# Apokleos/kata-xpu-device-plugin

Measured on AMD Instinct MI355X. Metric: Allocate() p50 latency, lower is better.
Workload: dtype n/a; 1 GPU; model=kata-xpu-device-plugin-amd pod-churn, node=8x MI355X (mock sysfs, vfio-pci), gpus_per_pod=1, discovered_gpus=8, concurrent_clients=1, parallelism=1 churn client(s), one plugin daemon

## Files before the change

### kata_xpu_device_plugin_amd/config.py

```python
from __future__ import annotations

import argparse
import dataclasses
import os
from dataclasses import dataclass, field
from typing import Optional, Sequence

STRATEGY_CDI_CRI = "cdi-cri"
STRATEGY_CDI_ANNOTATIONS = "cdi-annotations"
STRATEGY_DEVICE_NODES = "device-nodes"
STRATEGIES = (STRATEGY_CDI_CRI, STRATEGY_CDI_ANNOTATIONS, STRATEGY_DEVICE_NODES)

DEFAULT_VENDOR_ALLOWLIST = (0x1002,)


def bundled_pci_ids_path() -> str:
    return os.path.join(os.path.dirname(os.path.abspath(__file__)),
                        "data", "pci.ids")


def _env(name: str, default: str) -> str:
    return os.environ.get(f"KXDP_{name}", default)


def _env_int(name: str, default: int) -> int:
    return int(os.environ.get(f"KXDP_{name}", default))


def _env_float(name: str, default: float) -> float:
    return float(os.environ.get(f"KXDP_{name}", default))


def _env_bool(name: str, default: bool) -> bool:
    raw = os.environ.get(f"KXDP_{name}")
    if raw is None:
        return default
    return raw.strip().lower() in ("1", "true", "yes", "on")


@dataclass
class Config:
    sysfs_root: str = field(default_factory=lambda: _env("SYSFS_ROOT", "/sys"))
    dev_root: str = field(default_factory=lambda: _env("DEV_ROOT", "/dev"))

    vendor_allowlist: Sequence[int] = field(
        default_factory=lambda: tuple(
            int(v, 16) for v in _env("VENDORS", "1002").split(",") if v
        )
    )
    device_allowlist: Sequence[int] = field(
        default_factory=lambda: tuple(
            int(v, 16) for v in _env("DEVICES", "").split(",") if v
        )
    )
    required_driver: str = field(default_factory=lambda: _env("DRIVER", "vfio-pci"))
    gpu_class_prefixes: Sequence[int] = (0x03, 0x12)

    resource_namespace: str = field(default_factory=lambda: _env("NAMESPACE", "amd.com"))
    pci_ids_paths: Sequence[str] = field(
        default_factory=lambda: tuple(
            p for p in _env(
                "PCI_IDS",
                bundled_pci_ids_path()
                + ":/usr/share/misc/pci.ids:/usr/share/hwdata/pci.ids:/usr/pci.ids",
            ).split(":")
            if p
        )
    )
    unified_resource_name: str = field(default_factory=lambda: _env("UNIFIED_RESOURCE", ""))

    cdi_dir: str = field(default_factory=lambda: _env("CDI_DIR", "/var/run/cdi"))
    cdi_kind: str = field(default_factory=lambda: _env("CDI_KIND", "amd.com/gpu"))
    cdi_spec_name: str = field(default_factory=lambda: _env("CDI_SPEC_NAME", "kxdp-vfio"))
    cdi_format: str = field(default_factory=lambda: _env("CDI_FORMAT", "yaml"))
    cdi_version: str = field(default_factory=lambda: _env("CDI_VERSION", "0.8.0"))
    device_list_strategy: str = field(default_factory=lambda: _env("STRATEGY", STRATEGY_CDI_CRI))

    kubelet_socket_dir: str = field(
        default_factory=lambda: _env("KUBELET_DIR", "/var/lib/kubelet/device-plugins")
    )
    kubelet_socket_name: str = "kubelet.sock"
    plugin_socket_prefix: str = field(default_factory=lambda: _env("SOCKET_PREFIX", "kata-xpu-amd"))
    registration_mode: str = field(default_factory=lambda: _env("REGISTRATION_MODE", "legacy"))
    plugins_registry_dir: str = field(
        default_factory=lambda: _env("PLUGINS_REGISTRY", "/var/lib/kubelet/plugins_registry")
    )
    grpc_timeout_s: float = field(default_factory=lambda: _env_float("GRPC_TIMEOUT_S", 5.0))

    topology_hint_path: str = field(
        default_factory=lambda: _env("TOPOLOGY_HINT", "/etc/kata-xpu-amd/topology.json")
    )

    health_poll_interval_s: float = field(default_factory=lambda: _env_float("HEALTH_POLL_S", 10.0))
    amdsmi_health: bool = field(default_factory=lambda: _env_bool("AMDSMI_HEALTH", True))
    reject_unhealthy: bool = field(default_factory=lambda: _env_bool("REJECT_UNHEALTHY", True))
    gpu_probe_interval_s: float = field(default_factory=lambda: _env_float("GPU_PROBE_S", 0.0))
    rescan_interval_s: float = field(default_factory=lambda: _env_float("RESCAN_S", 0.0))

    rpc_timing_path: str = field(default_factory=lambda: _env("RPC_TIMING", ""))

    gc_tuning: bool = field(default_factory=lambda: _env_bool("GC_TUNING", True))
    cpu_affinity: str = field(default_factory=lambda: _env("CPU_AFFINITY", ""))

    metrics_port: int = field(default_factory=lambda: _env_int("METRICS_PORT", 0))
    log_level: str = field(default_factory=lambda: _env("LOG_LEVEL", "INFO"))

    native: str = field(default_factory=lambda: _env("NATIVE", "auto"))
    grpc_server: str = field(default_factory=lambda: _env("GRPC_SERVER", "auto"))

    def validate(self) -> None:
        if self.device_list_strategy not in STRATEGIES:
            raise ValueError(
                f"device_list_strategy must be one of {STRATEGIES}, "
                f"got {self.device_list_strategy!r}"
            )
        if self.cdi_format not in ("yaml", "json"):
            raise ValueError(f"cdi_format must be yaml|json, got {self.cdi_format!r}")
        from .cdi.schema import KNOWN_CDI_VERSIONS
        if self.cdi_version not in KNOWN_CDI_VERSIONS:
            raise ValueError(
                f"cdi_version must be one of {KNOWN_CDI_VERSIONS}, "
                f"got {self.cdi_version!r}")
        if "/" not in self.cdi_kind:
            raise ValueError(f"cdi_kind must look like vendor/class, got {self.cdi_kind!r}")
        if self.native not in ("auto", "require", "off"):
            raise ValueError(f"native must be auto|require|off, got {self.native!r}")
        if self.grpc_server not in ("auto", "native", "aio"):
            raise ValueError(
                f"grpc_server must be auto|native|aio, got {self.grpc_server!r}")
        if self.registration_mode not in ("legacy", "watcher", "both"):
            raise ValueError(
                f"registration_mode must be legacy|watcher|both, "
                f"got {self.registration_mode!r}")

    @property
    def kubelet_socket(self) -> str:
        return os.path.join(self.kubelet_socket_dir, self.kubelet_socket_name)

    @classmethod
    def add_args(cls, parser: argparse.ArgumentParser) -> None:
        g = parser.add_argument_group("plugin config (env: KXDP_*)")
        g.add_argument("--sysfs-root", dest="sysfs_root")
        g.add_argument("--dev-root", dest="dev_root")
        g.add_argument("--cdi-dir", dest="cdi_dir")
        g.add_argument("--cdi-kind", dest="cdi_kind")
        g.add_argument("--strategy", dest="device_list_strategy", choices=STRATEGIES)
        g.add_argument("--kubelet-dir", dest="kubelet_socket_dir")
        g.add_argument("--namespace", dest="resource_namespace")
        g.add_argument("--driver", dest="required_driver")
        g.add_argument("--topology-hint", dest="topology_hint_path")
        g.add_argument("--metrics-port", dest="metrics_port", type=int)
        g.add_argument("--log-level", dest="log_level")
        g.add_argument("--native", dest="native", choices=("auto", "require", "off"))
        g.add_argument("--grpc-server", dest="grpc_server",
                       choices=("auto", "native", "aio"))
        g.add_argument("--registration-mode", dest="registration_mode",
                       choices=("legacy", "watcher", "both"))
        g.add_argument("--plugins-registry", dest="plugins_registry_dir")
        g.add_argument("--unified-resource", dest="unified_resource_name")
        g.add_argument("--cdi-format", dest="cdi_format", choices=("yaml", "json"))
        g.add_argument("--gpu-probe-interval", dest="gpu_probe_interval_s",
                       type=float)

    @classmethod
    def from_args(cls, args: Optional[argparse.Namespace] = None) -> "Config":
        cfg = cls()
        if args is not None:
            for f in dataclasses.fields(cls):
                v = getattr(args, f.name, None)
                if v is not None:
                    setattr(cfg, f.name, v)
        cfg.validate()
        return cfg
```

### kata_xpu_device_plugin_amd/plugin/server.py

```python
from __future__ import annotations

import asyncio
import atexit
import os
import threading
import time
import weakref
from typing import Dict, List, Optional

import grpc
import grpc.aio

from ..cdi.spec import ANNOTATION_PREFIX, qualified_name
from ..config import Config, STRATEGY_CDI_ANNOTATIONS, STRATEGY_CDI_CRI
from ..discovery.sysfs import read_hex, read_link_base
from ..topology.hive import GPUTopology, preferred_sets
from ..utils.log import get_logger
from . import api
from .state import DeviceState

log = get_logger(__name__)

try:
    from .. import _native as _NATIVE
except ImportError:
    _NATIVE = None

ENV_CDI_VENDOR_CLASS = "KUBERNETES_CDI_VENDOR_CLASS"
ENV_PCI_RESOURCE_PREFIX = "PCI_RESOURCE_"

_DEVICE_PLUGIN_PATH = "/v1beta1.DevicePlugin/"

_LIVE_NATIVE = weakref.WeakSet()


@atexit.register
def _stop_native_servers() -> None:
    for plugin in list(_LIVE_NATIVE):
        srv = plugin._native_server
        if srv is not None:
            try:
                srv.stop(0.0)
            except Exception:
                pass


def _stream_open() -> None:
    """DeviceState subscription of one open native ListAndWatch stream."""


def native_server_available() -> bool:
    return _NATIVE is not None and hasattr(_NATIVE, "GrpcServer")


class AllocationError(Exception):
    pass


class XPUDevicePlugin:

    def __init__(
        self,
        cfg: Config,
        resource_name: str,
        state: DeviceState,
        topo: GPUTopology,
        socket_name: Optional[str] = None,
    ):
        self.cfg = cfg
        self.resource_name = resource_name
        self.state = state
        self.topo = topo
        short = resource_name.split("/", 1)[1].lower()
        self.socket_name = socket_name or f"{cfg.plugin_socket_prefix}-{short}.sock"
        self.socket_path = os.path.join(cfg.kubelet_socket_dir, self.socket_name)
        self._aio_server: Optional[grpc.aio.Server] = None
        self._loop: Optional[asyncio.AbstractEventLoop] = None
        self._thread: Optional[threading.Thread] = None
        self._stop = threading.Event()
        self._serving = threading.Event()
        self._lifecycle = threading.Lock()
        self._removal_lock = threading.Lock()
        self._expected_removals = 0
        self.watcher_servicer = None
        self.watcher_socket_path: Optional[str] = None
        self._allocations = 0
        self._allocate_failures = 0
        self._last_allocate_s = 0.0
        self._allocate_seconds_total = 0.0
        self._native_server = None
        self._native_unsubscribe = None
        self._stream_subscriptions: List = []
        self._devices_dir = os.path.join(cfg.sysfs_root, "bus", "pci", "devices")
        self._vendor_list = list(cfg.vendor_allowlist)
        self._qn_cache: Dict[str, str] = {}
        self._bdf_cache = None
        self._timing = {"allocate_us": [], "preferred_us": [],
                        "loop_lag_us": []} if cfg.rpc_timing_path else None
        self._env_res_name = ENV_PCI_RESOURCE_PREFIX + resource_name.upper(
        ).replace("/", "_").replace(".", "_").replace("-", "_")

    def _native_stats(self):
        srv = self._native_server
        return srv.stats() if srv is not None else (0, 0, None, 0.0)

    @property
    def allocations(self) -> int:
        return self._allocations + self._native_stats()[0]

    @allocations.setter
    def allocations(self, v: int) -> None:
        self._allocations = v

    @property
    def allocate_failures(self) -> int:
        return self._allocate_failures + self._native_stats()[1]

    @allocate_failures.setter
    def allocate_failures(self, v: int) -> None:
        self._allocate_failures = v

    @property
    def last_allocate_s(self) -> float:
        last = self._native_stats()[2]
        return self._last_allocate_s if not last else last

    @last_allocate_s.setter
    def last_allocate_s(self, v: float) -> None:
        self._last_allocate_s = v

    @property
    def allocate_seconds_total(self) -> float:
        return self._allocate_seconds_total + self._native_stats()[3]

    @allocate_seconds_total.setter
    def allocate_seconds_total(self, v: float) -> None:
        self._allocate_seconds_total = v

    def _qn(self, gid: str) -> str:
        qn = self._qn_cache.get(gid)
        if qn is None:
            qn = self._qn_cache[gid] = qualified_name(self.cfg.cdi_kind, gid)
        return qn

    async def GetDevicePluginOptions(self, request, context):
        return api.DevicePluginOptions(
            pre_start_required=False,
            get_preferred_allocation_available=True,
        )

    def _device_list(self, snapshot=None) -> List[object]:
        devs = []
        if snapshot is None:
            snapshot = self.state.snapshot()
        for dev, healthy in snapshot:
            d = api.Device(
                id=dev.id,
                health=api.HEALTHY if healthy else api.UNHEALTHY,
            )
            if dev.numa_node >= 0:
                d.topology.nodes.add(id=dev.numa_node)
            devs.append(d)
        return devs

    async def ListAndWatch(self, request, context):
        loop = asyncio.get_running_loop()
        event = asyncio.Event()

        def _notify() -> None:
            try:
                loop.call_soon_threadsafe(event.set)
            except RuntimeError:
                pass

        unsubscribe = self.state.subscribe(_notify)
        try:
            yield api.ListAndWatchResponse(devices=self._device_list())
            while not self._stop.is_set():
                await event.wait()
                event.clear()
                if self._stop.is_set():
                    break
                yield api.ListAndWatchResponse(devices=self._device_list())
        finally:
            unsubscribe()

    def _revalidate_many(self, ids: List[str]) -> None:
        groups = []
        for gid in ids:
            dev = self.state.device(gid)
            if dev is None:
                raise AllocationError(f"unknown device id {gid}")
            if self.cfg.reject_unhealthy and not self.state.is_healthy(gid):
                raise AllocationError(f"device {gid} is Unhealthy")
            groups.append((gid, [fn.bdf for fn in dev.functions]))
        if self.cfg.native != "off":
            if _NATIVE is None and self.cfg.native == "require":
                raise RuntimeError("_native extension required but missing")
            if _NATIVE is not None:
                err = _NATIVE.revalidate_groups(
                    self._devices_dir, groups,
                    self._vendor_list, self.cfg.required_driver,
                )
                if err:
                    raise AllocationError(err)
                return
        for gid, _bdfs in groups:
            self._revalidate_py(gid)

    def _revalidate_py(self, gid: str) -> None:
        dev = self.state.device(gid)
        assert dev is not None
        devices_dir = self._devices_dir
        for fn in dev.functions:
            p = os.path.join(devices_dir, fn.bdf)
            if read_link_base(os.path.join(p, "iommu_group")) != gid:
                raise AllocationError(f"device {fn.bdf} no longer in IOMMU group {gid}")
            vendor = read_hex(os.path.join(p, "vendor"))
            if vendor not in set(self.cfg.vendor_allowlist):
                raise AllocationError(f"device {fn.bdf} vendor {vendor:#x} not allowed")
            if read_link_base(os.path.join(p, "driver")) != self.cfg.required_driver:
                raise AllocationError(
                    f"device {fn.bdf} not bound to {self.cfg.required_driver}"
                )

    def _container_response(self, ids: List[str]):
        resp = api.ContainerAllocateResponse()
        strategy = self.cfg.device_list_strategy
        bdfs: List[str] = []
        if ids and strategy not in (STRATEGY_CDI_CRI, STRATEGY_CDI_ANNOTATIONS):
            vfio_ctl = os.path.join(self.cfg.dev_root, "vfio", "vfio")
            resp.devices.add(
                container_path=vfio_ctl, host_path=vfio_ctl, permissions="rw"
            )
        for gid in ids:
            dev = self.state.device(gid)
            assert dev is not None
            bdfs.extend(dev.bdfs)
            if strategy == STRATEGY_CDI_CRI:
                resp.cdi_devices.add(name=self._qn(gid))
            elif strategy == STRATEGY_CDI_ANNOTATIONS:
                key = f"{ANNOTATION_PREFIX}vfio{gid}"
                resp.annotations[key] = self._qn(gid)
            else:
                path = os.path.join(self.cfg.dev_root, dev.vfio_node)
                resp.devices.add(
                    container_path=path, host_path=path, permissions="rw"
                )
        if strategy in (STRATEGY_CDI_CRI, STRATEGY_CDI_ANNOTATIONS):
            resp.envs[ENV_CDI_VENDOR_CLASS] = self.cfg.cdi_kind
        resp.envs[self._env_res_name] = ",".join(bdfs)
        return resp

    async def Allocate(self, request, context):
        t0 = time.perf_counter()
        response = api.AllocateResponse()
        try:
            for creq in request.container_requests:
                ids = list(creq.devices_ids)
                self._revalidate_many(ids)
                response.container_responses.append(self._container_response(ids))
        except AllocationError as e:
            self.allocate_failures += 1
            log.warning("Allocate(%s) rejected: %s", self.resource_name, e)
            await context.abort(grpc.StatusCode.INVALID_ARGUMENT, str(e))
        self.allocations += 1
        self.last_allocate_s = time.perf_counter() - t0
        self.allocate_seconds_total += self.last_allocate_s
        if self._timing is not None:
            self._timing["allocate_us"].append(self.last_allocate_s * 1e6)
        return response

    async def GetPreferredAllocation(self, request, context):
        return self._preferred_allocation(request)

    def _preferred_allocation(self, request):
        t0 = time.perf_counter() if self._timing is not None else 0.0
        resp = api.PreferredAllocationResponse()
        gen = self.state.generation
        cached = self._bdf_cache
        if cached is not None and cached[0] == gen:
            bdf_of = cached[1]
        else:
            bdf_of = self.state.bdf_map()
            self._bdf_cache = (gen, bdf_of)
        for creq in request.container_requests:
            available = [d for d in creq.available_device_ids if d in bdf_of]
            must = list(creq.must_include_device_ids)
            pick = preferred_sets(
                self.topo, bdf_of, available, must, creq.allocation_size
            )
            resp.container_responses.add(device_ids=pick)
        if self._timing is not None:
            self._timing["preferred_us"].append(
                (time.perf_counter() - t0) * 1e6)
        return resp

    async def PreStartContainer(self, request, context):
        return api.PreStartContainerResponse()

    def start(self, register: bool = True) -> None:
        with self._lifecycle:
            self._start_locked(register)

    def _use_native_server(self) -> bool:
        want = self.cfg.grpc_server
        if want == "aio":
            return False
        if native_server_available() and self.cfg.native != "off":
            return True
        if want == "native":
            raise RuntimeError(
                "grpc_server=native needs the _native extension "
                "(and native != off)")
        if self.cfg.native == "require":
            raise RuntimeError("_native extension required but missing")
        return False

    def _start_locked(self, register: bool) -> None:
        self._stop.clear()
        if self._use_native_server():
            self._start_native()
        else:
            self._start_aio()
        ch = grpc.insecure_channel(f"unix://{self.socket_path}")
        try:
            grpc.channel_ready_future(ch).result(timeout=self.cfg.grpc_timeout_s)
        finally:
            ch.close()
        self._serving.set()
        if register and self.cfg.registration_mode in ("legacy", "both"):
            try:
                self.register_with_kubelet()
            except Exception as e:
                log.warning("kubelet registration failed (%s); serving "
                            "anyway and retrying in background", e)
                self._spawn_registration_retry()
        log.info("plugin %s serving on %s (%s registration)",
                 self.resource_name, self.socket_path,
                 self.cfg.registration_mode)

    def _start_aio(self) -> None:
        self._loop_ready = threading.Event()
        self._start_error: Optional[BaseException] = None
        self._thread = threading.Thread(
            target=self._serve_thread,
            name=f"kxdp-grpc-{self.resource_name.split('/')[-1]}",
            daemon=True,
        )
        self._thread.start()
        if not self._loop_ready.wait(self.cfg.grpc_timeout_s):
            raise RuntimeError(f"gRPC server for {self.resource_name} "
                               "did not start in time")
        if self._start_error is not None:
            self._thread.join(timeout=2.0)
            raise self._start_error

    def _start_native(self) -> None:
        os.makedirs(self.cfg.kubelet_socket_dir, exist_ok=True)
        if os.path.exists(self.socket_path):
            self._note_expected_removal()
            os.unlink(self.socket_path)
        paths = [self.socket_path]
        if self.cfg.registration_mode in ("watcher", "both"):
            from .watcher_registration import (
                SERVICE_PATH_PREFIX,
                WatcherRegistrationServicer,
            )
            os.makedirs(self.cfg.plugins_registry_dir, exist_ok=True)
            self.watcher_servicer = WatcherRegistrationServicer(
                self.resource_name, self.socket_path)
            self.watcher_socket_path = os.path.join(
                self.cfg.plugins_registry_dir, self.socket_name)
            if os.path.exists(self.watcher_socket_path):
                os.unlink(self.watcher_socket_path)
            paths.append(self.watcher_socket_path)
        srv = _NATIVE.GrpcServer(paths)
        p = _DEVICE_PLUGIN_PATH
        srv.register_constant(
            p + "GetDevicePluginOptions",
            api.DevicePluginOptions(
                pre_start_required=False,
                get_preferred_allocation_available=True,
            ).SerializeToString())
        srv.register_constant(
            p + "PreStartContainer",
            api.PreStartContainerResponse().SerializeToString())
        srv.register_watch(p + "ListAndWatch", self._on_watch_streams)
        srv.register_unary(p + "GetPreferredAllocation",
                           self._preferred_allocation_bytes)
        srv.configure_allocate(
            p + "Allocate",
            strategy=self.cfg.device_list_strategy,
            reject_unhealthy=bool(self.cfg.reject_unhealthy),
            cdi_kind=self.cfg.cdi_kind,
            env_name=self._env_res_name,
            dev_root=self.cfg.dev_root,
            devices_dir=self._devices_dir,
            vendors=self._vendor_list,
            required_driver=self.cfg.required_driver,
            on_reject=self._log_rejection,
            timing=self._timing is not None,
        )
        if self.watcher_servicer is not None and len(paths) > 1:
            srv.register_unary(SERVICE_PATH_PREFIX + "GetInfo",
                               self.watcher_servicer.get_info_bytes)
            srv.register_unary(
                SERVICE_PATH_PREFIX + "NotifyRegistrationStatus",
                self.watcher_servicer.notify_registration_status_bytes)
        self._native_server = srv
        self._native_unsubscribe = self.state.subscribe_snapshot(
            self._push_native_state)
        try:
            srv.start()
        except BaseException:
            self._native_unsubscribe()
            self._native_unsubscribe = None
            self._native_server = None
            raise
        _LIVE_NATIVE.add(self)

    def _push_native_state(self, snapshot, generation) -> None:
        srv = self._native_server
        if srv is None:
            return
        dev_root = self.cfg.dev_root
        rows = []
        for dev, healthy in snapshot:
            qn = self._qn(dev.id)
            rows.append((
                dev.id,
                [fn.bdf for fn in dev.functions],
                bool(healthy),
                api.CDIDevice(name=qn).SerializeToString(),
                f"{ANNOTATION_PREFIX}vfio{dev.id}",
                qn,
                os.path.join(dev_root, dev.vfio_node),
            ))
        srv.update_table(rows)
        srv.publish(api.ListAndWatchResponse(
            devices=self._device_list(snapshot)).SerializeToString())

    def _on_watch_streams(self, delta: int) -> None:
        subs = self._stream_subscriptions
        for _ in range(delta):
            subs.append(self.state.subscribe(_stream_open))
        for _ in range(-delta):
            if subs:
                subs.pop()()

    def _preferred_allocation_bytes(self, request: bytes) -> bytes:
        return self._preferred_allocation(
            api.PreferredAllocationRequest.FromString(request)
        ).SerializeToString()

    def _log_rejection(self, err: str) -> None:
        log.warning("Allocate(%s) rejected: %s", self.resource_name, err)

    def _stop_native(self) -> None:
        srv = self._native_server
        if srv is None:
            return
        if self._native_unsubscribe is not None:
            self._native_unsubscribe()
            self._native_unsubscribe = None
        srv.stop(1.0)
        n, fails, last, total = srv.stats()
        if self._timing is not None:
            self._timing["allocate_us"] = list(srv.allocate_timing_us())
            self._timing["loop_lag_us"] = []
            self._dump_timing()
        self._native_server = None
        _LIVE_NATIVE.discard(self)
        while self._stream_subscriptions:
            self._stream_subscriptions.pop()()
        self._allocations += n
        self._allocate_failures += fails
        self._allocate_seconds_total += total
        if last:
            self._last_allocate_s = last

    def _spawn_registration_retry(self) -> None:
        def retry():
            delay = 1.0
            while self._serving.is_set() and not self._stop.is_set():
                if self._stop.wait(delay):
                    return
                if not self._serving.is_set():
                    return
                try:
                    self.register_with_kubelet()
                    log.info("kubelet registration succeeded after retry")
                    return
                except Exception:
                    delay = min(delay * 2, 30.0)

        threading.Thread(target=retry, daemon=True,
                         name=f"kxdp-register-retry-{self.socket_name}").start()

    def _serve_thread(self) -> None:
        loop = asyncio.new_event_loop()
        self._loop = loop
        asyncio.set_event_loop(loop)

        async def _main():
            server = grpc.aio.server(
                options=[("grpc.max_concurrent_streams", 64),
                         ("grpc.optimization_target", "latency")])
            api.add_device_plugin_servicer(server, self)
            os.makedirs(self.cfg.kubelet_socket_dir, exist_ok=True)
            if os.path.exists(self.socket_path):
                self._note_expected_removal()
                os.unlink(self.socket_path)
            server.add_insecure_port(f"unix://{self.socket_path}")
            if self.cfg.registration_mode in ("watcher", "both"):
                from .watcher_registration import (
                    WatcherRegistrationServicer,
                    add_watcher_registration_servicer,
                )
                os.makedirs(self.cfg.plugins_registry_dir, exist_ok=True)
                self.watcher_servicer = WatcherRegistrationServicer(
                    self.resource_name, self.socket_path)
                self.watcher_socket_path = os.path.join(
                    self.cfg.plugins_registry_dir, self.socket_name)
                add_watcher_registration_servicer(server, self.watcher_servicer)
                if os.path.exists(self.watcher_socket_path):
                    os.unlink(self.watcher_socket_path)
                server.add_insecure_port(f"unix://{self.watcher_socket_path}")
            await server.start()
            self._aio_server = server
            self._stop_async = asyncio.Event()
            lag_task = None
            if self._timing is not None:
                async def _lag_monitor():
                    while not self._stop_async.is_set():
                        t0 = time.perf_counter()
                        await asyncio.sleep(0.001)
                        lag = (time.perf_counter() - t0 - 0.001) * 1e6
                        self._timing["loop_lag_us"].append(max(0.0, lag))
                        if len(self._timing["loop_lag_us"]) > 200_000:
                            del self._timing["loop_lag_us"][:100_000]
                lag_task = asyncio.ensure_future(_lag_monitor())
            self._loop_ready.set()
            await self._stop_async.wait()
            if lag_task is not None:
                lag_task.cancel()
            await server.stop(grace=1.0)
            if self._timing is not None:
                self._dump_timing()

        try:
            loop.run_until_complete(_main())
        except BaseException as e:
            self._start_error = e
            self._loop_ready.set()
        finally:
            try:
                loop.close()
            except Exception:
                pass

    def _dump_timing(self) -> None:
        import json
        import statistics as stats

        def dist(xs):
            if not xs:
                return None
            xs = sorted(xs)
            n = len(xs)
            return {"n": n,
                    "p50": round(xs[n // 2], 1),
                    "p90": round(xs[min(n - 1, int(n * 0.9))], 1),
                    "p99": round(xs[min(n - 1, int(n * 0.99))], 1),
                    "max": round(xs[-1], 1),
                    "mean": round(stats.fmean(xs), 1)}

        out = {k: dist(v) for k, v in self._timing.items()}
        path = f"{self.cfg.rpc_timing_path}.{self.socket_name}.json"
        try:
            with open(path, "w") as f:
                json.dump(out, f, indent=1)
            log.info("rpc timing breakdown → %s", path)
        except OSError as e:
            log.warning("could not write rpc timing: %s", e)

    def register_with_kubelet(self) -> None:
        ch = grpc.insecure_channel(f"unix://{self.cfg.kubelet_socket}")
        try:
            grpc.channel_ready_future(ch).result(timeout=self.cfg.grpc_timeout_s)
            stub = api.RegistrationStub(ch)
            stub.Register(
                api.RegisterRequest(
                    version=api.VERSION,
                    endpoint=self.socket_name,
                    resource_name=self.resource_name,
                    options=api.DevicePluginOptions(
                        pre_start_required=False,
                        get_preferred_allocation_available=True,
                    ),
                ),
                timeout=self.cfg.grpc_timeout_s,
            )
        finally:
            ch.close()

    def stop(self) -> None:
        with self._lifecycle:
            self._stop_locked()

    def _stop_locked(self) -> None:
        self._stop.set()
        self._serving.clear()
        self.state.poke()
        if os.path.exists(self.socket_path):
            self._note_expected_removal()
        self._stop_native()
        if self._loop is not None and getattr(self, "_stop_async", None) is not None:
            try:
                self._loop.call_soon_threadsafe(self._stop_async.set)
            except RuntimeError:
                pass
        if self._thread is not None:
            self._thread.join(timeout=5.0)
            self._thread = None
        self._aio_server = None
        self._loop = None
        for path in (self.socket_path,
                     getattr(self, "watcher_socket_path", None)):
            if path and os.path.exists(path):
                try:
                    os.unlink(path)
                except OSError:
                    pass

    def restart(self, register: bool = True) -> None:
        self.stop()
        self.start(register=register)

    def _note_expected_removal(self) -> None:
        with self._removal_lock:
            self._expected_removals += 1

    def consume_expected_removal(self) -> bool:
        with self._removal_lock:
            if self._expected_removals > 0:
                self._expected_removals -= 1
                return True
            return False

    @property
    def serving(self) -> bool:
        return self._serving.is_set()
```

### native/xpu_grpc_server.cpp

```cpp
#include <pybind11/pybind11.h>
#include <pybind11/stl.h>

#include <atomic>
#include <cerrno>
#include <chrono>
#include <cstring>
#include <fcntl.h>
#include <memory>
#include <mutex>
#include <poll.h>
#include <stdexcept>
#include <sys/epoll.h>
#include <sys/eventfd.h>
#include <sys/socket.h>
#include <sys/uio.h>
#include <sys/un.h>
#include <thread>
#include <unistd.h>
#include <unordered_map>

#include "h2.h"
#include "pbwire.h"

namespace py = pybind11;
using namespace kxdp;

namespace {

constexpr int STRATEGY_CDI_CRI = 0;
constexpr int STRATEGY_CDI_ANNOTATIONS = 1;
constexpr int STRATEGY_DEVICE_NODES = 2;
constexpr size_t kMaxTimingSamples = 1u << 20;

struct DeviceEntry {
    std::vector<std::string> bdfs;
    bool healthy = true;
    std::string cdi_device;
    std::string ann_key, ann_value;
    std::string dev_path;
};

using Table = std::unordered_map<std::string, DeviceEntry>;

struct AllocateConfig {
    bool enabled = false;
    std::string path;
    int strategy = STRATEGY_CDI_CRI;
    bool reject_unhealthy = true;
    std::string cdi_kind, env_name, dev_root, devices_dir, required_driver;
    std::vector<long> vendors;
    bool timing = false;
};

enum class Kind { CONSTANT, WATCH, PYTHON, ALLOCATE };

struct Method {
    Kind kind;
    std::string bytes;
    py::object fn;
};

std::string link_base(int dirfd, const char* name) {
    char buf[512];
    ssize_t n = ::readlinkat(dirfd, name, buf, sizeof(buf) - 1);
    if (n <= 0) return {};
    buf[n] = 0;
    const char* slash = std::strrchr(buf, '/');
    return std::string(slash ? slash + 1 : buf);
}

long read_vendor(int dirfd) {
    int fd = ::openat(dirfd, "vendor", O_RDONLY | O_CLOEXEC);
    if (fd < 0) return -1;
    char buf[64];
    ssize_t n = ::read(fd, buf, sizeof(buf) - 1);
    ::close(fd);
    if (n <= 0) return -1;
    buf[n] = 0;
    errno = 0;
    char* end = nullptr;
    long v = std::strtol(buf, &end, 16);
    if (errno || end == buf) return -1;
    return v;
}

struct IoConn {
    int fd;
    h2::Conn h2;
    size_t woff = 0;
    size_t watching = 0;
    bool want_write = false;
    IoConn(int f, h2::App* app) : fd(f), h2(app) {}
};

class GrpcServer : public h2::App {
public:
    explicit GrpcServer(std::vector<std::string> paths)
        : paths_(std::move(paths)) {}

    ~GrpcServer() override {
        if (thread_.joinable()) {
            py::gil_scoped_release rel;
            request_stop(0.0);
            thread_.join();
        }
        methods_.clear();
        on_reject_ = py::object();
        on_watch_change_ = py::object();
    }

    void register_constant(const std::string& path, const std::string& bytes) {
        check_not_running();
        methods_[path] = Method{Kind::CONSTANT, bytes, py::object()};
    }
    void register_watch(const std::string& path, py::object on_change) {
        check_not_running();
        methods_[path] = Method{Kind::WATCH, {}, py::object()};
        on_watch_change_ = std::move(on_change);
    }
    void register_unary(const std::string& path, py::object fn) {
        check_not_running();
        methods_[path] = Method{Kind::PYTHON, {}, std::move(fn)};
    }
    void configure_allocate(const std::string& path, const std::string& strategy,
                            bool reject_unhealthy, const std::string& cdi_kind,
                            const std::string& env_name,
                            const std::string& dev_root,
                            const std::string& devices_dir,
                            const std::vector<long>& vendors,
                            const std::string& required_driver,
                            py::object on_reject, bool timing) {
        check_not_running();
        alloc_.enabled = true;
        alloc_.path = path;
        alloc_.strategy = strategy == "cdi-cri" ? STRATEGY_CDI_CRI
                          : strategy == "cdi-annotations" ? STRATEGY_CDI_ANNOTATIONS
                          : STRATEGY_DEVICE_NODES;
        alloc_.reject_unhealthy = reject_unhealthy;
        alloc_.cdi_kind = cdi_kind;
        alloc_.env_name = env_name;
        alloc_.dev_root = dev_root;
        alloc_.devices_dir = devices_dir;
        alloc_.vendors = vendors;
        alloc_.required_driver = required_driver;
        alloc_.timing = timing;
        on_reject_ = std::move(on_reject);
        methods_[path] = Method{Kind::ALLOCATE, {}, py::object()};
    }

    void update_table(const std::vector<std::tuple<
            std::string, std::vector<std::string>, bool, py::bytes,
            std::string, std::string, std::string>>& devices) {
        auto t = std::make_shared<Table>();
        for (auto& d : devices) {
            DeviceEntry e;
            e.bdfs = std::get<1>(d);
            e.healthy = std::get<2>(d);
            e.cdi_device = std::string(std::get<3>(d));
            e.ann_key = std::get<4>(d);
            e.ann_value = std::get<5>(d);
            e.dev_path = std::get<6>(d);
            (*t)[std::get<0>(d)] = std::move(e);
        }
        std::lock_guard<std::mutex> g(table_mu_);
        table_ = std::move(t);
    }

    void publish(const std::string& message) {
        auto m = std::make_shared<const std::string>(message);
        {
            std::lock_guard<std::mutex> g(pub_mu_);
            latest_ = std::move(m);
            pub_gen_++;
        }
        wake();
    }

    void start() {
        if (thread_.joinable()) throw std::runtime_error("server already started");
        stop_.store(false);
        ep_ = ::epoll_create1(EPOLL_CLOEXEC);
        wake_fd_ = ::eventfd(0, EFD_NONBLOCK | EFD_CLOEXEC);
        if (ep_ < 0 || wake_fd_ < 0) {
            close_fds();
            throw std::runtime_error("epoll/eventfd setup failed");
        }
        add_epoll(wake_fd_, EPOLLIN);
        for (auto& path : paths_) {
            sockaddr_un addr{};
            addr.sun_family = AF_UNIX;
            if (path.size() >= sizeof(addr.sun_path)) {
                close_fds();
                throw std::runtime_error("socket path too long: " + path);
            }
            std::memcpy(addr.sun_path, path.c_str(), path.size() + 1);
            int fd = ::socket(AF_UNIX, SOCK_STREAM | SOCK_NONBLOCK | SOCK_CLOEXEC, 0);
            if (fd < 0 || ::bind(fd, (sockaddr*)&addr, sizeof(addr)) < 0 ||
                ::listen(fd, 128) < 0) {
                std::string why = std::strerror(errno);
                if (fd >= 0) ::close(fd);
                close_fds();
                throw std::runtime_error("cannot listen on " + path + ": " + why);
            }
            listeners_.push_back(fd);
            bound_.push_back(path);
            add_epoll(fd, EPOLLIN);
        }
        thread_ = std::thread([this] { run(); });
    }

    void stop(double grace) {
        if (!thread_.joinable()) return;
        py::gil_scoped_release rel;
        request_stop(grace);
        thread_.join();
    }

    bool running() const { return thread_.joinable(); }

    py::tuple stats() {
        std::lock_guard<std::mutex> g(stat_mu_);
        return py::make_tuple(allocations_, failures_, last_s_, total_s_);
    }

    std::vector<double> allocate_timing_us() {
        std::lock_guard<std::mutex> g(stat_mu_);
        return alloc_us_;
    }

    void on_rpc(h2::Conn& c, uint32_t sid, const std::string& path,
                std::string& msg) override {
        auto it = methods_.find(path);
        if (it == methods_.end())
            return c.reply_error(sid, h2::GRPC_UNIMPLEMENTED, "Method not found!");
        Method& m = it->second;
        switch (m.kind) {
        case Kind::CONSTANT:
            return c.reply_unary(sid, m.bytes);
        case Kind::ALLOCATE:
            return handle_allocate(c, sid, msg);
        case Kind::WATCH: {
            std::shared_ptr<const std::string> latest;
            {
                std::lock_guard<std::mutex> g(pub_mu_);
                latest = latest_;
            }
            c.start_stream(sid);
            if (latest) c.push_message(sid, *latest);
            return;
        }
        case Kind::PYTHON:
            return handle_python(c, sid, m, msg);
        }
    }

private:
    void check_not_running() {
        if (thread_.joinable())
            throw std::runtime_error("register methods before start()");
    }

    void wake() {
        if (wake_fd_ >= 0) {
            uint64_t one = 1;
            ssize_t r = ::write(wake_fd_, &one, sizeof(one));
            (void)r;
        }
    }

    void request_stop(double grace) {
        grace_s_ = grace;
        stop_.store(true);
        wake();
    }

    void add_epoll(int fd, uint32_t events) {
        epoll_event ev{};
        ev.events = events;
        ev.data.fd = fd;
        ::epoll_ctl(ep_, EPOLL_CTL_ADD, fd, &ev);
    }

    void close_fds() {
        for (int fd : listeners_) ::close(fd);
        listeners_.clear();
        for (auto& p : bound_) ::unlink(p.c_str());
        bound_.clear();
        if (wake_fd_ >= 0) ::close(wake_fd_);
        if (ep_ >= 0) ::close(ep_);
        wake_fd_ = ep_ = -1;
        if (dirfd_ >= 0) ::close(dirfd_);
        dirfd_ = -1;
        dirfd_table_ = nullptr;
    }

    struct GilHold {
        PyThreadState*& ts;
        bool held = false;
        explicit GilHold(PyThreadState*& t) : ts(t) {
            if (ts && !_Py_IsFinalizing()) {
                PyEval_RestoreThread(ts);
                held = true;
            }
        }
        ~GilHold() {
            if (held) ts = PyEval_SaveThread();
        }
    };

    void handle_python(h2::Conn& c, uint32_t sid, Method& m, std::string& msg) {
        bool ok = false;
        int status = h2::GRPC_UNKNOWN;
        std::string payload;
        {
            GilHold gil(ts_);
            if (!gil.held) {
                status = h2::GRPC_UNAVAILABLE;
                payload = "server shutting down";
            } else {
                try {
                    py::object r = m.fn(py::bytes(msg));
                    if (py::isinstance<py::bytes>(r)) {
                        payload = r.cast<std::string>();
                        ok = true;
                    } else {
                        auto t = r.cast<std::pair<int, std::string>>();
                        status = t.first;
                        payload = t.second;
                    }
                } catch (py::error_already_set& e) {
                    try {
                        payload = "Unexpected " +
                                  py::str(e.type()).cast<std::string>() + ": " +
                                  py::str(e.value()).cast<std::string>();
                    } catch (...) {
                        payload = "handler raised";
                    }
                    e.restore();
                    PyErr_Clear();
                } catch (std::exception& e) {
                    payload = e.what();
                }
            }
        }
        if (ok) c.reply_unary(sid, payload);
        else c.reply_error(sid, status, payload);
    }

    void report_watchers(IoConn& io, size_t now) {
        if (now == io.watching) return;
        long delta = (long)now - (long)io.watching;
        io.watching = now;
        GilHold gil(ts_);
        if (!gil.held || !on_watch_change_ || on_watch_change_.is_none()) return;
        try {
            on_watch_change_(delta);
        } catch (py::error_already_set& e) {
            e.restore();
            PyErr_Clear();
        }
    }

    void log_rejection(const std::string& err) {
        GilHold gil(ts_);
        if (!gil.held || !on_reject_ || on_reject_.is_none()) return;
        try {
            on_reject_(err);
        } catch (py::error_already_set& e) {
            e.restore();
            PyErr_Clear();
        }
    }

    bool open_devices_dir() {
        if (dirfd_ >= 0) ::close(dirfd_);
        dirfd_ = ::open(alloc_.devices_dir.c_str(),
                        O_RDONLY | O_DIRECTORY | O_CLOEXEC);
        return dirfd_ >= 0;
    }

    std::string revalidate(const std::string& gid, const DeviceEntry& dev) {
        for (const auto& bdf : dev.bdfs) {
            const int flags = O_RDONLY | O_DIRECTORY | O_CLOEXEC;
            int dfd = ::openat(dirfd_, bdf.c_str(), flags);
            if (dfd < 0) {
                if (!open_devices_dir())
                    return "cannot open " + alloc_.devices_dir;
                dfd = ::openat(dirfd_, bdf.c_str(), flags);
            }
            if (dfd < 0) return "device " + bdf + " vanished";
            std::string err;
            if (link_base(dfd, "iommu_group") != gid) {
                err = "device " + bdf + " no longer in IOMMU group " + gid;
            } else {
                long vendor = read_vendor(dfd);
                if (vendor < 0 ||
                    std::find(alloc_.vendors.begin(), alloc_.vendors.end(),
                              vendor) == alloc_.vendors.end())
                    err = "device " + bdf + " vendor not allowed";
                else if (link_base(dfd, "driver") != alloc_.required_driver)
                    err = "device " + bdf + " not bound to " +
                          alloc_.required_driver;
            }
            ::close(dfd);
            if (!err.empty()) return err;
        }
        return {};
    }

    std::string allocate_container(const Table& table,
                                   const std::vector<std::string>& ids,
                                   std::string& out) {
        std::vector<const DeviceEntry*> devs;
        devs.reserve(ids.size());
        for (const auto& gid : ids) {
            auto it = table.find(gid);
            if (it == table.end()) return "unknown device id " + gid;
            if (alloc_.reject_unhealthy && !it->second.healthy)
                return "device " + gid + " is Unhealthy";
            devs.push_back(&it->second);
        }
        if (dirfd_ < 0 || dirfd_table_ != &table) {
            if (!open_devices_dir()) return "cannot open " + alloc_.devices_dir;
            dirfd_table_ = &table;
        }
        for (size_t i = 0; i < ids.size(); i++) {
            std::string err = revalidate(ids[i], *devs[i]);
            if (!err.empty()) return err;
        }
        const bool cdi = alloc_.strategy != STRATEGY_DEVICE_NODES;
        std::string bdfs;
        for (auto* d : devs)
            for (const auto& b : d->bdfs) {
                if (!bdfs.empty()) bdfs.push_back(',');
                bdfs += b;
            }
        static const std::string kVendorClass = "KUBERNETES_CDI_VENDOR_CLASS";
        if (cdi && alloc_.env_name == kVendorClass) {
            pb::put_map_entry(out, 1, alloc_.env_name, bdfs);
        } else if (cdi && kVendorClass < alloc_.env_name) {
            pb::put_map_entry(out, 1, kVendorClass, alloc_.cdi_kind);
            pb::put_map_entry(out, 1, alloc_.env_name, bdfs);
        } else {
            pb::put_map_entry(out, 1, alloc_.env_name, bdfs);
            if (cdi) pb::put_map_entry(out, 1, kVendorClass, alloc_.cdi_kind);
        }
        if (!cdi) {
            auto spec = [&](const std::string& path) {
                std::string s;
                pb::put_bytes(s, 1, path);
                pb::put_bytes(s, 2, path);
                pb::put_bytes(s, 3, "rw", 2);
                pb::put_bytes(out, 3, s);
            };
            if (!ids.empty()) spec(alloc_.dev_root + "/vfio/vfio");
            for (auto* d : devs) spec(d->dev_path);
        }
        if (alloc_.strategy == STRATEGY_CDI_ANNOTATIONS)
            for (auto* d : devs)
                pb::put_map_entry(out, 4, d->ann_key, d->ann_value);
        if (alloc_.strategy == STRATEGY_CDI_CRI)
            for (auto* d : devs) pb::put_bytes(out, 5, d->cdi_device);
        return {};
    }

    void handle_allocate(h2::Conn& c, uint32_t sid, const std::string& msg) {
        auto t0 = std::chrono::steady_clock::now();
        std::shared_ptr<const Table> table;
        {
            std::lock_guard<std::mutex> g(table_mu_);
            table = table_;
        }
        std::vector<std::vector<std::string>> reqs;
        if (!pb::parse_allocate_request(msg, reqs))
            return c.reply_error(sid, h2::GRPC_INTERNAL,
                                 "Exception deserializing request!");
        static const Table kEmpty;
        const Table& tbl = table ? *table : kEmpty;
        std::string resp, err;
        for (const auto& ids : reqs) {
            std::string cresp;
            err = allocate_container(tbl, ids, cresp);
            if (!err.empty()) break;
            pb::put_bytes(resp, 1, cresp);
        }
        if (!err.empty()) {
            {
                std::lock_guard<std::mutex> g(stat_mu_);
                failures_++;
            }
            c.reply_error(sid, h2::GRPC_INVALID_ARGUMENT, err);
            log_rejection(err);
            return;
        }
        double dt = std::chrono::duration<double>(
                        std::chrono::steady_clock::now() - t0).count();
        {
            std::lock_guard<std::mutex> g(stat_mu_);
            allocations_++;
            last_s_ = dt;
            total_s_ += dt;
            if (alloc_.timing && alloc_us_.size() < kMaxTimingSamples)
                alloc_us_.push_back(dt * 1e6);
        }
        c.reply_unary(sid, resp);
    }

    void set_want_write(IoConn& io, bool on) {
        if (io.want_write == on) return;
        io.want_write = on;
        epoll_event ev{};
        ev.events = EPOLLIN | (on ? EPOLLOUT : 0);
        ev.data.fd = io.fd;
        ::epoll_ctl(ep_, EPOLL_CTL_MOD, io.fd, &ev);
    }

    bool flush(IoConn& io) {
        std::string& out = io.h2.out();
        while (io.woff < out.size()) {
            iovec iov{(void*)(out.data() + io.woff), out.size() - io.woff};
            msghdr mh{};
            mh.msg_iov = &iov;
            mh.msg_iovlen = 1;
            ssize_t n = ::sendmsg(io.fd, &mh, MSG_NOSIGNAL);
            if (n < 0) {
                if (errno == EINTR) continue;
                if (errno == EAGAIN || errno == EWOULDBLOCK) {
                    set_want_write(io, true);
                    return true;
                }
                return false;
            }
            io.woff += (size_t)n;
        }
        out.clear();
        io.woff = 0;
        set_want_write(io, false);
        return !io.h2.want_close();
    }

    void close_conn(int fd) {
        auto it = conns_.find(fd);
        if (it == conns_.end()) return;
        report_watchers(*it->second, 0);
        ::epoll_ctl(ep_, EPOLL_CTL_DEL, fd, nullptr);
        ::close(fd);
        conns_.erase(it);
    }

    void on_readable(IoConn& io) {
        ssize_t n = ::read(io.fd, rbuf_, sizeof(rbuf_));
        if (n == 0) return close_conn(io.fd);
        if (n < 0) {
            if (errno == EAGAIN || errno == EINTR) return;
            return close_conn(io.fd);
        }
        io.h2.feed((const uint8_t*)rbuf_, (size_t)n);
        report_watchers(io, io.h2.watch_streams());
        if (!flush(io)) close_conn(io.fd);
    }

    void deliver_publications() {
        std::shared_ptr<const std::string> latest;
        uint64_t gen;
        {
            std::lock_guard<std::mutex> g(pub_mu_);
            latest = latest_;
            gen = pub_gen_;
        }
        if (gen == pub_seen_ || !latest) return;
        pub_seen_ = gen;
        std::vector<int> done;
        for (auto& kv : conns_) {
            kv.second->h2.broadcast(*latest);
            if (!flush(*kv.second)) done.push_back(kv.first);
        }
        for (int fd : done) close_conn(fd);
    }

    void shutdown_connections() {
        for (int fd : listeners_) ::close(fd);
        listeners_.clear();
        for (auto& p : bound_) ::unlink(p.c_str());
        bound_.clear();
        for (auto& kv : conns_) kv.second->h2.begin_shutdown();
        auto deadline = std::chrono::steady_clock::now() +
                        std::chrono::duration<double>(grace_s_);
        for (auto& kv : conns_) {
            IoConn& io = *kv.second;
            while (flush(io) && io.woff < io.h2.out().size()) {
                auto left = std::chrono::duration_cast<std::chrono::milliseconds>(
                    deadline - std::chrono::steady_clock::now()).count();
                if (left <= 0) break;
                pollfd p{io.fd, POLLOUT, 0};
                if (::poll(&p, 1, (int)left) <= 0) break;
            }
            ::shutdown(io.fd, SHUT_WR);
            while (::read(io.fd, rbuf_, sizeof(rbuf_)) > 0) {}
            report_watchers(io, 0);
            ::close(io.fd);
        }
        conns_.clear();
    }

    void run() {
        PyGILState_STATE gstate = PyGILState_Ensure();
        ts_ = PyEval_SaveThread();
        epoll_event evs[64];
        while (!stop_.load()) {
            int n = ::epoll_wait(ep_, evs, 64, -1);
            if (n < 0) {
                if (errno == EINTR) continue;
                break;
            }
            for (int i = 0; i < n && !stop_.load(); i++) {
                int fd = evs[i].data.fd;
                if (fd == wake_fd_) {
                    uint64_t v;
                    while (::read(wake_fd_, &v, sizeof(v)) > 0) {}
                    deliver_publications();
                    continue;
                }
                if (std::find(listeners_.begin(), listeners_.end(), fd) !=
                    listeners_.end()) {
                    for (;;) {
                        int cfd = ::accept4(fd, nullptr, nullptr,
                                            SOCK_NONBLOCK | SOCK_CLOEXEC);
                        if (cfd < 0) break;
                        auto io = std::make_unique<IoConn>(cfd, this);
                        IoConn& ref = *io;
                        conns_[cfd] = std::move(io);
                        add_epoll(cfd, EPOLLIN);
                        if (!flush(ref)) close_conn(cfd);
                    }
                    continue;
                }
                auto it = conns_.find(fd);
                if (it == conns_.end()) continue;
                IoConn& io = *it->second;
                if (evs[i].events & EPOLLOUT) {
                    if (!flush(io)) {
                        close_conn(fd);
                        continue;
                    }
                }
                if (evs[i].events & (EPOLLIN | EPOLLHUP | EPOLLERR))
                    on_readable(io);
            }
        }
        shutdown_connections();
        if (!_Py_IsFinalizing()) {
            PyEval_RestoreThread(ts_);
            PyGILState_Release(gstate);
        }
        ts_ = nullptr;
        int ep = ep_, wfd = wake_fd_;
        ep_ = wake_fd_ = -1;
        ::close(ep);
        ::close(wfd);
        if (dirfd_ >= 0) ::close(dirfd_);
        dirfd_ = -1;
        dirfd_table_ = nullptr;
    }

    std::vector<std::string> paths_, bound_;
    std::unordered_map<std::string, Method> methods_;
    AllocateConfig alloc_;
    py::object on_reject_, on_watch_change_;

    std::mutex table_mu_;
    std::shared_ptr<const Table> table_;
    std::mutex pub_mu_;
    std::shared_ptr<const std::string> latest_;
    uint64_t pub_gen_ = 0;
    uint64_t pub_seen_ = 0;

    std::mutex stat_mu_;
    uint64_t allocations_ = 0, failures_ = 0;
    double last_s_ = 0.0, total_s_ = 0.0;
    std::vector<double> alloc_us_;

    std::thread thread_;
    std::atomic<bool> stop_{false};
    double grace_s_ = 1.0;
    int ep_ = -1, wake_fd_ = -1;
    std::vector<int> listeners_;
    std::unordered_map<int, std::unique_ptr<IoConn>> conns_;
    PyThreadState* ts_ = nullptr;
    int dirfd_ = -1;
    const Table* dirfd_table_ = nullptr;
    char rbuf_[65536];
};

}

void kxdp_init_grpc_server(py::module_& m) {
    py::class_<GrpcServer>(m, "GrpcServer")
        .def(py::init<std::vector<std::string>>(), py::arg("socket_paths"))
        .def("register_constant", &GrpcServer::register_constant,
             py::arg("path"), py::arg("response"))
        .def("register_watch", &GrpcServer::register_watch, py::arg("path"),
             py::arg("on_change") = py::none())
        .def("register_unary", &GrpcServer::register_unary, py::arg("path"),
             py::arg("fn"),
             "fn(request bytes) -> response bytes | (status code, message)")
        .def("configure_allocate", &GrpcServer::configure_allocate,
             py::arg("path"), py::arg("strategy"), py::arg("reject_unhealthy"),
             py::arg("cdi_kind"), py::arg("env_name"), py::arg("dev_root"),
             py::arg("devices_dir"), py::arg("vendors"),
             py::arg("required_driver"), py::arg("on_reject"),
             py::arg("timing") = false)
        .def("update_table", &GrpcServer::update_table, py::arg("devices"))
        .def("publish", &GrpcServer::publish, py::arg("message"))
        .def("start", &GrpcServer::start)
        .def("stop", &GrpcServer::stop, py::arg("grace") = 1.0)
        .def("stats", &GrpcServer::stats)
        .def("allocate_timing_us", &GrpcServer::allocate_timing_us)
        .def_property_readonly("running", &GrpcServer::running);
}
```

### setup.py

```python
import os
import subprocess
import sys

import pybind11

ROOT = os.path.dirname(os.path.abspath(__file__))
PKG = "kata_xpu_device_plugin_amd"


def build_hip(arch: str = "gfx950", verbose: bool = True) -> str:
    import sysconfig

    hipcc = os.environ.get("HIPCC", "/opt/rocm/bin/hipcc")
    src = os.path.join(ROOT, "probes", "xpu_probe.hip")
    ext = sysconfig.get_config_var("EXT_SUFFIX") or ".so"
    out = os.path.join(ROOT, PKG, f"_gpuprobe{ext}")
    if os.path.exists(out) and os.path.getmtime(out) > os.path.getmtime(src):
        return out
    cmd = [
        hipcc, f"--offload-arch={arch}", "-O3", "-std=c++17",
        "-fPIC", "-shared",
        "-x", "hip", src,
        f"-I{pybind11.get_include()}",
        f"-I{sysconfig.get_paths()['include']}",
        "-o", out,
    ]
    if verbose:
        print("+", " ".join(cmd), file=sys.stderr)
    subprocess.run(cmd, check=True)
    return out


if __name__ == "__main__" or "setuptools" in sys.modules:
    from setuptools import Extension, setup

    if __name__ == "__main__":
        setup(
            name="kata-xpu-device-plugin-amd",
            version="0.1.0",
            packages=[
                PKG, f"{PKG}.discovery", f"{PKG}.topology", f"{PKG}.cdi",
                f"{PKG}.plugin", f"{PKG}.health", f"{PKG}.utils",
                f"{PKG}.testing", f"{PKG}.tools",
            ],
            package_data={PKG: ["data/pci.ids"]},
            include_package_data=True,
            entry_points={
                "console_scripts": [
                    "kata-xpu-device-plugin-amd=kata_xpu_device_plugin_amd.plugin.manager:main",
                    "kxdp-topo=kata_xpu_device_plugin_amd.tools.topo:main",
                    "kxdp-burnin=kata_xpu_device_plugin_amd.tools.burnin:main",
                    "kxdp-bind=kata_xpu_device_plugin_amd.tools.bind:main",
                    "kxdp-sriov=kata_xpu_device_plugin_amd.tools.sriov:main",
                    "kxdp-validate=kata_xpu_device_plugin_amd.tools.validate:main",
                    "kxdp-ident=kata_xpu_device_plugin_amd.tools.ident:main",
                    "kxdp-doctor=kata_xpu_device_plugin_amd.tools.doctor:main",
                    "kxdp-assignments=kata_xpu_device_plugin_amd.tools.assignments:main",
                    "kxdp-resourceslice=kata_xpu_device_plugin_amd.tools.resourceslice:main",
                    "kxdp-partition=kata_xpu_device_plugin_amd.tools.partition:main",
                ],
            },
            ext_modules=[
                Extension(
                    f"{PKG}._native",
                    sources=["native/xpu_native.cpp",
                             "native/xpu_grpc_server.cpp"],
                    depends=["native/h2.h", "native/hpack.h",
                             "native/pbwire.h"],
                    include_dirs=[pybind11.get_include(), "native"],
                    extra_compile_args=["-O2", "-std=c++17"],
                    extra_link_args=["-pthread"],
                    language="c++",
                ),
            ],
        )
```

Baseline: 35.80 us.

## Run native gRPC server on a pool of epoll loop threads

Result: slower. 65.09 us (+81.8%).

```diff
diff --git a/kata_xpu_device_plugin_amd/config.py b/kata_xpu_device_plugin_amd/config.py
--- a/kata_xpu_device_plugin_amd/config.py
+++ b/kata_xpu_device_plugin_amd/config.py
@@ -12,6 +12,7 @@
 STRATEGIES = (STRATEGY_CDI_CRI, STRATEGY_CDI_ANNOTATIONS, STRATEGY_DEVICE_NODES)
 
 DEFAULT_VENDOR_ALLOWLIST = (0x1002,)
+DEFAULT_GRPC_LOOPS = 8
 
 
 def bundled_pci_ids_path() -> str:
@@ -107,8 +108,15 @@
 
     native: str = field(default_factory=lambda: _env("NATIVE", "auto"))
     grpc_server: str = field(default_factory=lambda: _env("GRPC_SERVER", "auto"))
+    grpc_loops: int = field(
+        default_factory=lambda: _env_int("GRPC_LOOPS", DEFAULT_GRPC_LOOPS))
 
     def validate(self) -> None:
+        if isinstance(self.grpc_loops, bool) or \
+                not isinstance(self.grpc_loops, int) or \
+                not 1 <= self.grpc_loops <= 8:
+            raise ValueError(
+                f"grpc_loops must be an integer 1..8, got {self.grpc_loops!r}")
         if self.device_list_strategy not in STRATEGIES:
             raise ValueError(
                 f"device_list_strategy must be one of {STRATEGIES}, "
@@ -154,6 +162,7 @@
         g.add_argument("--native", dest="native", choices=("auto", "require", "off"))
         g.add_argument("--grpc-server", dest="grpc_server",
                        choices=("auto", "native", "aio"))
+        g.add_argument("--grpc-loops", dest="grpc_loops", type=int)
         g.add_argument("--registration-mode", dest="registration_mode",
                        choices=("legacy", "watcher", "both"))
         g.add_argument("--plugins-registry", dest="plugins_registry_dir")
diff --git a/kata_xpu_device_plugin_amd/plugin/server.py b/kata_xpu_device_plugin_amd/plugin/server.py
--- a/kata_xpu_device_plugin_amd/plugin/server.py
+++ b/kata_xpu_device_plugin_amd/plugin/server.py
@@ -91,6 +91,7 @@
         self._native_server = None
         self._native_unsubscribe = None
         self._stream_subscriptions: List = []
+        self._stream_lock = threading.Lock()
         self._devices_dir = os.path.join(cfg.sysfs_root, "bus", "pci", "devices")
         self._vendor_list = list(cfg.vendor_allowlist)
         self._qn_cache: Dict[str, str] = {}
@@ -375,7 +376,7 @@
             if os.path.exists(self.watcher_socket_path):
                 os.unlink(self.watcher_socket_path)
             paths.append(self.watcher_socket_path)
-        srv = _NATIVE.GrpcServer(paths)
+        srv = _NATIVE.GrpcServer(paths, loops=self.cfg.grpc_loops)
         p = _DEVICE_PLUGIN_PATH
         srv.register_constant(
             p + "GetDevicePluginOptions",
@@ -443,11 +444,12 @@
 
     def _on_watch_streams(self, delta: int) -> None:
         subs = self._stream_subscriptions
-        for _ in range(delta):
-            subs.append(self.state.subscribe(_stream_open))
-        for _ in range(-delta):
-            if subs:
-                subs.pop()()
+        with self._stream_lock:
+            for _ in range(delta):
+                subs.append(self.state.subscribe(_stream_open))
+            for _ in range(-delta):
+                if subs:
+                    subs.pop()()
 
     def _preferred_allocation_bytes(self, request: bytes) -> bytes:
         return self._preferred_allocation(
@@ -472,8 +474,9 @@
             self._dump_timing()
         self._native_server = None
         _LIVE_NATIVE.discard(self)
-        while self._stream_subscriptions:
-            self._stream_subscriptions.pop()()
+        with self._stream_lock:
+            while self._stream_subscriptions:
+                self._stream_subscriptions.pop()()
         self._allocations += n
         self._allocate_failures += fails
         self._allocate_seconds_total += total
diff --git a/native/loop_pool.h b/native/loop_pool.h
--- /dev/null
+++ b/native/loop_pool.h
@@ -0,0 +1,730 @@
+#pragma once
+
+#include <algorithm>
+#include <atomic>
+#include <cerrno>
+#include <chrono>
+#include <cstdlib>
+#include <cstring>
+#include <fcntl.h>
+#include <functional>
+#include <memory>
+#include <mutex>
+#include <poll.h>
+#include <stdexcept>
+#include <string>
+#include <system_error>
+#include <sys/epoll.h>
+#include <sys/eventfd.h>
+#include <sys/socket.h>
+#include <sys/uio.h>
+#include <sys/un.h>
+#include <thread>
+#include <unistd.h>
+#include <unordered_map>
+#include <vector>
+
+#include "h2.h"
+#include "pbwire.h"
+
+namespace kxdp {
+
+constexpr int STRATEGY_CDI_CRI = 0;
+constexpr int STRATEGY_CDI_ANNOTATIONS = 1;
+constexpr int STRATEGY_DEVICE_NODES = 2;
+constexpr size_t kMaxTimingSamples = 1u << 20;
+constexpr int kMaxLoops = 8;
+
+struct DeviceEntry {
+    std::vector<std::string> bdfs;
+    bool healthy = true;
+    std::string cdi_device;
+    std::string ann_key, ann_value;
+    std::string dev_path;
+};
+
+using Table = std::unordered_map<std::string, DeviceEntry>;
+
+struct AllocateConfig {
+    bool enabled = false;
+    std::string path;
+    int strategy = STRATEGY_CDI_CRI;
+    bool reject_unhealthy = true;
+    std::string cdi_kind, env_name, dev_root, devices_dir, required_driver;
+    std::vector<long> vendors;
+    bool timing = false;
+};
+
+struct UnaryResult {
+    bool ok = false;
+    int status = h2::GRPC_UNKNOWN;
+    std::string payload;
+};
+
+struct Hooks {
+    std::function<void(int loop)> thread_begin, thread_end;
+    std::function<UnaryResult(int loop, const std::string& path,
+                              const std::string& msg)> unary;
+    std::function<void(int loop, long delta)> watch_change;
+    std::function<void(int loop, const std::string& err)> reject;
+};
+
+struct PoolStats {
+    uint64_t allocations = 0, failures = 0;
+    double last_s = 0.0, total_s = 0.0;
+};
+
+inline std::string link_base(int dirfd, const char* name) {
+    char buf[512];
+    ssize_t n = ::readlinkat(dirfd, name, buf, sizeof(buf) - 1);
+    if (n <= 0) return {};
+    buf[n] = 0;
+    const char* slash = std::strrchr(buf, '/');
+    return std::string(slash ? slash + 1 : buf);
+}
+
+inline long read_vendor(int dirfd) {
+    int fd = ::openat(dirfd, "vendor", O_RDONLY | O_CLOEXEC);
+    if (fd < 0) return -1;
+    char buf[64];
+    ssize_t n = ::read(fd, buf, sizeof(buf) - 1);
+    ::close(fd);
+    if (n <= 0) return -1;
+    buf[n] = 0;
+    errno = 0;
+    char* end = nullptr;
+    long v = std::strtol(buf, &end, 16);
+    if (errno || end == buf) return -1;
+    return v;
+}
+
+class LoopPool {
+    enum class Kind { CONSTANT, WATCH, CALLBACK, ALLOCATE };
+
+    struct Method {
+        Kind kind;
+        std::string bytes;
+    };
+
+    struct IoConn {
+        int fd;
+        h2::Conn h2;
+        size_t woff = 0;
+        size_t watching = 0;
+        bool want_write = false;
+        IoConn(int f, h2::App* app) : fd(f), h2(app) {}
+    };
+
+    struct Loop : h2::App {
+        LoopPool* pool = nullptr;
+        int index = 0;
+        std::thread thread;
+        bool started = false;
+        std::atomic<int> nconn{0};
+        std::mutex box_mu;
+        std::vector<int> inbox;
+        int wake_fd = -1;
+        int ep = -1;
+        std::unordered_map<int, std::unique_ptr<IoConn>> conns;
+        int dirfd = -1;
+        std::shared_ptr<const Table> dirfd_table;
+        uint64_t pub_seen = 0;
+        char rbuf[65536];
+
+        void on_rpc(h2::Conn& c, uint32_t sid, const std::string& path,
+                    std::string& msg) override {
+            pool->on_rpc(*this, c, sid, path, msg);
+        }
+    };
+
+public:
+    LoopPool(std::vector<std::string> paths, int loops)
+        : paths_(std::move(paths)) {
+        if (loops < 1 || loops > kMaxLoops)
+            throw std::invalid_argument("loops must be 1..8");
+        for (int i = 0; i < loops; i++) {
+            loops_.push_back(std::make_unique<Loop>());
+            loops_.back()->pool = this;
+            loops_.back()->index = i;
+        }
+    }
+
+    ~LoopPool() {
+        request_stop(0.0);
+        join();
+    }
+
+    LoopPool(const LoopPool&) = delete;
+    LoopPool& operator=(const LoopPool&) = delete;
+
+    void add_constant(const std::string& path, const std::string& bytes) {
+        check_not_running();
+        methods_[path] = Method{Kind::CONSTANT, bytes};
+    }
+    void add_watch(const std::string& path) {
+        check_not_running();
+        methods_[path] = Method{Kind::WATCH, {}};
+    }
+    void add_callback(const std::string& path) {
+        check_not_running();
+        methods_[path] = Method{Kind::CALLBACK, {}};
+    }
+    void set_allocate(AllocateConfig cfg) {
+        check_not_running();
+        alloc_ = std::move(cfg);
+        alloc_.enabled = true;
+        methods_[alloc_.path] = Method{Kind::ALLOCATE, {}};
+    }
+    void set_hooks(Hooks hooks) {
+        check_not_running();
+        hooks_ = std::move(hooks);
+    }
+
+    void update_table(std::shared_ptr<const Table> t) {
+        std::lock_guard<std::mutex> g(table_mu_);
+        table_ = std::move(t);
+    }
+
+    void publish(const std::string& message) {
+        auto m = std::make_shared<const std::string>(message);
+        {
+            std::lock_guard<std::mutex> g(pub_mu_);
+            latest_ = std::move(m);
+            pub_gen_++;
+        }
+        for (auto& l : loops_) wake(*l);
+    }
+
+    void start() {
+        if (running()) throw std::runtime_error("server already started");
+        stop_.store(false);
+        for (auto& l : loops_) {
+            l->ep = ::epoll_create1(EPOLL_CLOEXEC);
+            int wfd = ::eventfd(0, EFD_NONBLOCK | EFD_CLOEXEC);
+            {
+                std::lock_guard<std::mutex> g(l->box_mu);
+                l->wake_fd = wfd;
+            }
+            if (l->ep < 0 || wfd < 0) {
+                close_fds();
+                throw std::runtime_error("epoll/eventfd setup failed");
+            }
+            add_epoll(*l, wfd, EPOLLIN);
+        }
+        for (auto& path : paths_) {
+            sockaddr_un addr{};
+            addr.sun_family = AF_UNIX;
+            if (path.size() >= sizeof(addr.sun_path)) {
+                close_fds();
+                throw std::runtime_error("socket path too long: " + path);
+            }
+            std::memcpy(addr.sun_path, path.c_str(), path.size() + 1);
+            int fd = ::socket(AF_UNIX, SOCK_STREAM | SOCK_NONBLOCK | SOCK_CLOEXEC, 0);
+            if (fd < 0 || ::bind(fd, (sockaddr*)&addr, sizeof(addr)) < 0 ||
+                ::listen(fd, 128) < 0) {
+                std::string why = std::strerror(errno);
+                if (fd >= 0) ::close(fd);
+                close_fds();
+                throw std::runtime_error("cannot listen on " + path + ": " + why);
+            }
+            listeners_.push_back(fd);
+            bound_.push_back(path);
+            add_epoll(*loops_[0], fd, EPOLLIN);
+        }
+        spawn(*loops_[0]);
+    }
+
+    void request_stop(double grace) {
+        if (!running()) return;
+        grace_s_.store(grace);
+        stop_.store(true);
+        for (auto& l : loops_) wake(*l);
+    }
+
+    void join() {
+        for (auto& l : loops_)
+            if (l->thread.joinable()) l->thread.join();
+        close_fds();
+    }
+
+    void stop(double grace) {
+        request_stop(grace);
+        join();
+    }
+
+    bool running() const { return loops_[0]->thread.joinable(); }
+    int loops() const { return (int)loops_.size(); }
+
+    PoolStats stats() {
+        std::lock_guard<std::mutex> g(stat_mu_);
+        return stat_;
+    }
+
+    std::vector<double> allocate_timing_us() {
+        std::lock_guard<std::mutex> g(stat_mu_);
+        return alloc_us_;
+    }
+
+    std::vector<int> loop_connections() const {
+        std::vector<int> out;
+        for (auto& l : loops_) out.push_back(l->nconn.load());
+        return out;
+    }
+
+private:
+    void check_not_running() {
+        if (running())
+            throw std::runtime_error("register methods before start()");
+    }
+
+    void wake(Loop& l) {
+        std::lock_guard<std::mutex> g(l.box_mu);
+        if (l.wake_fd >= 0) {
+            uint64_t one = 1;
+            ssize_t r = ::write(l.wake_fd, &one, sizeof(one));
+            (void)r;
+        }
+    }
+
+    void spawn(Loop& l) {
+        Loop* lp = &l;
+        l.started = true;
+        l.thread = std::thread([this, lp] { run(*lp); });
+    }
+
+    static void add_epoll(Loop& l, int fd, uint32_t events) {
+        epoll_event ev{};
+        ev.events = events;
+        ev.data.fd = fd;
+        ::epoll_ctl(l.ep, EPOLL_CTL_ADD, fd, &ev);
+    }
+
+    void close_fds() {
+        for (int fd : listeners_) ::close(fd);
+        listeners_.clear();
+        for (auto& p : bound_) ::unlink(p.c_str());
+        bound_.clear();
+        for (auto& l : loops_) {
+            std::vector<int> late;
+            int wfd;
+            {
+                std::lock_guard<std::mutex> g(l->box_mu);
+                wfd = l->wake_fd;
+                l->wake_fd = -1;
+                late.swap(l->inbox);
+            }
+            for (int fd : late) ::close(fd);
+            if (wfd >= 0) ::close(wfd);
+            if (l->ep >= 0) ::close(l->ep);
+            l->ep = -1;
+            if (l->dirfd >= 0) ::close(l->dirfd);
+            l->dirfd = -1;
+            l->dirfd_table.reset();
+            l->nconn.store(0);
+            l->started = false;
+        }
+    }
+
+    void on_rpc(Loop& l, h2::Conn& c, uint32_t sid, const std::string& path,
+                std::string& msg) {
+        auto it = methods_.find(path);
+        if (it == methods_.end())
+            return c.reply_error(sid, h2::GRPC_UNIMPLEMENTED, "Method not found!");
+        const Method& m = it->second;
+        switch (m.kind) {
+        case Kind::CONSTANT:
+            return c.reply_unary(sid, m.bytes);
+        case Kind::ALLOCATE:
+            return handle_allocate(l, c, sid, msg);
+        case Kind::WATCH: {
+            std::shared_ptr<const std::string> latest;
+            {
+                std::lock_guard<std::mutex> g(pub_mu_);
+                latest = latest_;
+            }
+            c.start_stream(sid);
+            if (latest) c.push_message(sid, *latest);
+            return;
+        }
+        case Kind::CALLBACK: {
+            UnaryResult r;
+            if (hooks_.unary) {
+                r = hooks_.unary(l.index, path, msg);
+            } else {
+                r.status = h2::GRPC_UNIMPLEMENTED;
+                r.payload = "Method not found!";
+            }
+            if (r.ok) c.reply_unary(sid, r.payload);
+            else c.reply_error(sid, r.status, r.payload);
+            return;
+        }
+        }
+    }
+
+    void report_watchers(Loop& l, IoConn& io, size_t now) {
+        if (now == io.watching) return;
+        long delta = (long)now - (long)io.watching;
+        io.watching = now;
+        if (hooks_.watch_change) hooks_.watch_change(l.index, delta);
+    }
+
+    bool open_devices_dir(Loop& l) {
+        if (l.dirfd >= 0) ::close(l.dirfd);
+        l.dirfd = ::open(alloc_.devices_dir.c_str(),
+                         O_RDONLY | O_DIRECTORY | O_CLOEXEC);
+        return l.dirfd >= 0;
+    }
+
+    std::string revalidate(Loop& l, const std::string& gid,
+                           const DeviceEntry& dev) {
+        for (const auto& bdf : dev.bdfs) {
+            const int flags = O_RDONLY | O_DIRECTORY | O_CLOEXEC;
+            int dfd = ::openat(l.dirfd, bdf.c_str(), flags);
+            if (dfd < 0) {
+                if (!open_devices_dir(l))
+                    return "cannot open " + alloc_.devices_dir;
+                dfd = ::openat(l.dirfd, bdf.c_str(), flags);
+            }
+            if (dfd < 0) return "device " + bdf + " vanished";
+            std::string err;
+            if (link_base(dfd, "iommu_group") != gid) {
+                err = "device " + bdf + " no longer in IOMMU group " + gid;
+            } else {
+                long vendor = read_vendor(dfd);
+                if (vendor < 0 ||
+                    std::find(alloc_.vendors.begin(), alloc_.vendors.end(),
+                              vendor) == alloc_.vendors.end())
+                    err = "device " + bdf + " vendor not allowed";
+                else if (link_base(dfd, "driver") != alloc_.required_driver)
+                    err = "device " + bdf + " not bound to " +
+                          alloc_.required_driver;
+            }
+            ::close(dfd);
+            if (!err.empty()) return err;
+        }
+        return {};
+    }
+
+    std::string allocate_container(Loop& l,
+                                   const std::shared_ptr<const Table>& held,
+                                   const Table& table,
+                                   const std::vector<std::string>& ids,
+                                   std::string& out) {
+        std::vector<const DeviceEntry*> devs;
+        devs.reserve(ids.size());
+        for (const auto& gid : ids) {
+            auto it = table.find(gid);
+            if (it == table.end()) return "unknown device id " + gid;
+            if (alloc_.reject_unhealthy && !it->second.healthy)
+                return "device " + gid + " is Unhealthy";
+            devs.push_back(&it->second);
+        }
+        if (l.dirfd < 0 || l.dirfd_table != held) {
+            if (!open_devices_dir(l)) return "cannot open " + alloc_.devices_dir;
+            l.dirfd_table = held;
+        }
+        for (size_t i = 0; i < ids.size(); i++) {
+            std::string err = revalidate(l, ids[i], *devs[i]);
+            if (!err.empty()) return err;
+        }
+        const bool cdi = alloc_.strategy != STRATEGY_DEVICE_NODES;
+        std::string bdfs;
+        for (auto* d : devs)
+            for (const auto& b : d->bdfs) {
+                if (!bdfs.empty()) bdfs.push_back(',');
+                bdfs += b;
+            }
+        static const std::string kVendorClass = "KUBERNETES_CDI_VENDOR_CLASS";
+        if (cdi && alloc_.env_name == kVendorClass) {
+            pb::put_map_entry(out, 1, alloc_.env_name, bdfs);
+        } else if (cdi && kVendorClass < alloc_.env_name) {
+            pb::put_map_entry(out, 1, kVendorClass, alloc_.cdi_kind);
+            pb::put_map_entry(out, 1, alloc_.env_name, bdfs);
+        } else {
+            pb::put_map_entry(out, 1, alloc_.env_name, bdfs);
+            if (cdi) pb::put_map_entry(out, 1, kVendorClass, alloc_.cdi_kind);
+        }
+        if (!cdi) {
+            auto spec = [&](const std::string& path) {
+                std::string s;
+                pb::put_bytes(s, 1, path);
+                pb::put_bytes(s, 2, path);
+                pb::put_bytes(s, 3, "rw", 2);
+                pb::put_bytes(out, 3, s);
+            };
+            if (!ids.empty()) spec(alloc_.dev_root + "/vfio/vfio");
+            for (auto* d : devs) spec(d->dev_path);
+        }
+        if (alloc_.strategy == STRATEGY_CDI_ANNOTATIONS)
+            for (auto* d : devs)
+                pb::put_map_entry(out, 4, d->ann_key, d->ann_value);
+        if (alloc_.strategy == STRATEGY_CDI_CRI)
+            for (auto* d : devs) pb::put_bytes(out, 5, d->cdi_device);
+        return {};
+    }
+
+    void handle_allocate(Loop& l, h2::Conn& c, uint32_t sid,
+                         const std::string& msg) {
+        auto t0 = std::chrono::steady_clock::now();
+        std::shared_ptr<const Table> table;
+        {
+            std::lock_guard<std::mutex> g(table_mu_);
+            table = table_;
+        }
+        std::vector<std::vector<std::string>> reqs;
+        if (!pb::parse_allocate_request(msg, reqs))
+            return c.reply_error(sid, h2::GRPC_INTERNAL,
+                                 "Exception deserializing request!");
+        static const Table kEmpty;
+        const Table& tbl = table ? *table : kEmpty;
+        std::string resp, err;
+        for (const auto& ids : reqs) {
+            std::string cresp;
+            err = allocate_container(l, table, tbl, ids, cresp);
+            if (!err.empty()) break;
+            pb::put_bytes(resp, 1, cresp);
+        }
+        if (!err.empty()) {
+            {
+                std::lock_guard<std::mutex> g(stat_mu_);
+                stat_.failures++;
+            }
+            c.reply_error(sid, h2::GRPC_INVALID_ARGUMENT, err);
+            if (hooks_.reject) hooks_.reject(l.index, err);
+            return;
+        }
+        double dt = std::chrono::duration<double>(
+                        std::chrono::steady_clock::now() - t0).count();
+        {
+            std::lock_guard<std::mutex> g(stat_mu_);
+            stat_.allocations++;
+            stat_.last_s = dt;
+            stat_.total_s += dt;
+            if (alloc_.timing && alloc_us_.size() < kMaxTimingSamples)
+                alloc_us_.push_back(dt * 1e6);
+        }
+        c.reply_unary(sid, resp);
+    }
+
+    static void set_want_write(Loop& l, IoConn& io, bool on) {
+        if (io.want_write == on) return;
+        io.want_write = on;
+        epoll_event ev{};
+        ev.events = on ? (EPOLLIN | EPOLLOUT) : EPOLLIN;
+        ev.data.fd = io.fd;
+        ::epoll_ctl(l.ep, EPOLL_CTL_MOD, io.fd, &ev);
+    }
+
+    static bool flush(Loop& l, IoConn& io) {
+        std::string& out = io.h2.out();
+        while (io.woff < out.size()) {
+            iovec iov{(void*)(out.data() + io.woff), out.size() - io.woff};
+            msghdr mh{};
+            mh.msg_iov = &iov;
+            mh.msg_iovlen = 1;
+            ssize_t n = ::sendmsg(io.fd, &mh, MSG_NOSIGNAL);
+            if (n < 0) {
+                if (errno == EINTR) continue;
+                if (errno == EAGAIN || errno == EWOULDBLOCK) {
+                    set_want_write(l, io, true);
+                    return true;
+                }
+                return false;
+            }
+            io.woff += (size_t)n;
+        }
+        out.clear();
+        io.woff = 0;
+        set_want_write(l, io, false);
+        return !io.h2.want_close();
+    }
+
+    void close_conn(Loop& l, int fd) {
+        auto it = l.conns.find(fd);
+        if (it == l.conns.end()) return;
+        report_watchers(l, *it->second, 0);
+        ::epoll_ctl(l.ep, EPOLL_CTL_DEL, fd, nullptr);
+        ::close(fd);
+        l.conns.erase(it);
+        l.nconn.fetch_sub(1);
+    }
+
+    void adopt(Loop& l, int cfd) {
+        auto io = std::make_unique<IoConn>(cfd, &l);
+        IoConn& ref = *io;
+        l.conns[cfd] = std::move(io);
+        add_epoll(l, cfd, EPOLLIN);
+        if (!flush(l, ref)) close_conn(l, cfd);
+    }
+
+    void drain_inbox(Loop& l) {
+        std::vector<int> fds;
+        {
+            std::lock_guard<std::mutex> g(l.box_mu);
+            fds.swap(l.inbox);
+        }
+        for (int fd : fds) adopt(l, fd);
+    }
+
+    void accept_all(Loop& l0, int lfd) {
+        for (;;) {
+            int cfd = ::accept4(lfd, nullptr, nullptr,
+                                SOCK_NONBLOCK | SOCK_CLOEXEC);
+            if (cfd < 0) break;
+            Loop* target = &l0;
+            int least = l0.nconn.load();
+            for (size_t i = 1; i < loops_.size(); i++) {
+                int n = loops_[i]->nconn.load();
+                if (n < least) {
+                    least = n;
+                    target = loops_[i].get();
+                }
+            }
+            if (!target->started) {
+                try {
+                    spawn(*target);
+                } catch (const std::system_error&) {
+                    target->started = false;
+                    target = &l0;
+                }
+            }
+            target->nconn.fetch_add(1);
+            if (target == &l0) {
+                adopt(l0, cfd);
+                continue;
+            }
+            {
+                std::lock_guard<std::mutex> g(target->box_mu);
+                target->inbox.push_back(cfd);
+            }
+            wake(*target);
+        }
+    }
+
+    void on_readable(Loop& l, IoConn& io) {
+        ssize_t n = ::read(io.fd, l.rbuf, sizeof(l.rbuf));
+        if (n == 0) return close_conn(l, io.fd);
+        if (n < 0) {
+            if (errno == EAGAIN || errno == EINTR) return;
+            return close_conn(l, io.fd);
+        }
+        io.h2.feed((const uint8_t*)l.rbuf, (size_t)n);
+        report_watchers(l, io, io.h2.watch_streams());
+        if (!flush(l, io)) close_conn(l, io.fd);
+    }
+
+    void deliver_publications(Loop& l) {
+        std::shared_ptr<const std::string> latest;
+        uint64_t gen;
+        {
+            std::lock_guard<std::mutex> g(pub_mu_);
+            latest = latest_;
+            gen = pub_gen_;
+        }
+        if (gen == l.pub_seen || !latest) return;
+        l.pub_seen = gen;
+        std::vector<int> done;
+        for (auto& kv : l.conns) {
+            kv.second->h2.broadcast(*latest);
+            if (!flush(l, *kv.second)) done.push_back(kv.first);
+        }
+        for (int fd : done) close_conn(l, fd);
+    }
+
+    void shutdown_connections(Loop& l) {
+        if (l.index == 0) {
+            for (int fd : listeners_) ::close(fd);
+            listeners_.clear();
+            for (auto& p : bound_) ::unlink(p.c_str());
+            bound_.clear();
+        }
+        drain_inbox(l);
+        for (auto& kv : l.conns) kv.second->h2.begin_shutdown();
+        auto deadline = std::chrono::steady_clock::now() +
+                        std::chrono::duration<double>(grace_s_.load());
+        for (auto& kv : l.conns) {
+            IoConn& io = *kv.second;
+            while (flush(l, io) && io.woff < io.h2.out().size()) {
+                auto left = std::chrono::duration_cast<std::chrono::milliseconds>(
+                    deadline - std::chrono::steady_clock::now()).count();
+                if (left <= 0) break;
+                pollfd p{io.fd, POLLOUT, 0};
+                if (::poll(&p, 1, (int)left) <= 0) break;
+            }
+            ::shutdown(io.fd, SHUT_WR);
+            while (::read(io.fd, l.rbuf, sizeof(l.rbuf)) > 0) {}
+            report_watchers(l, io, 0);
+            ::close(io.fd);
+            l.nconn.fetch_sub(1);
+        }
+        l.conns.clear();
+    }
+
+    void run(Loop& l) {
+        if (hooks_.thread_begin) hooks_.thread_begin(l.index);
+        int wake_fd;
+        {
+            std::lock_guard<std::mutex> g(l.box_mu);
+            wake_fd = l.wake_fd;
+        }
+        epoll_event evs[64];
+        while (!stop_.load()) {
+            int n = ::epoll_wait(l.ep, evs, 64, -1);
+            if (n < 0) {
+                if (errno == EINTR) continue;
+                break;
+            }
+            for (int i = 0; i < n && !stop_.load(); i++) {
+                int fd = evs[i].data.fd;
+                if (fd == wake_fd) {
+                    uint64_t v;
+                    while (::read(wake_fd, &v, sizeof(v)) > 0) {}
+                    drain_inbox(l);
+                    deliver_publications(l);
+                    continue;
+                }
+                if (l.index == 0 &&
+                    std::find(listeners_.begin(), listeners_.end(), fd) !=
+                        listeners_.end()) {
+                    accept_all(l, fd);
+                    continue;
+                }
+                auto it = l.conns.find(fd);
+                if (it == l.conns.end()) continue;
+                IoConn& io = *it->second;
+                if (evs[i].events & EPOLLOUT) {
+                    if (!flush(l, io)) {
+                        close_conn(l, fd);
+                        continue;
+                    }
+                }
+                if (evs[i].events & (EPOLLIN | EPOLLHUP | EPOLLERR))
+                    on_readable(l, io);
+            }
+        }
+        shutdown_connections(l);
+        if (hooks_.thread_end) hooks_.thread_end(l.index);
+    }
+
+    std::vector<std::string> paths_, bound_;
+    std::unordered_map<std::string, Method> methods_;
+    AllocateConfig alloc_;
+    Hooks hooks_;
+    std::vector<std::unique_ptr<Loop>> loops_;
+    std::vector<int> listeners_;
+
+    std::mutex table_mu_;
+    std::shared_ptr<const Table> table_;
+    std::mutex pub_mu_;
+    std::shared_ptr<const std::string> latest_;
+    uint64_t pub_gen_ = 0;
+
+    std::mutex stat_mu_;
+    PoolStats stat_;
+    std::vector<double> alloc_us_;
+
+    std::atomic<bool> stop_{false};
+    std::atomic<double> grace_s_{1.0};
+};
+
+}
diff --git a/native/xpu_grpc_server.cpp b/native/xpu_grpc_server.cpp
--- a/native/xpu_grpc_server.cpp
+++ b/native/xpu_grpc_server.cpp
@@ -1,126 +1,83 @@
 #include <pybind11/pybind11.h>
 #include <pybind11/stl.h>
 
-#include <atomic>
-#include <cerrno>
-#include <chrono>
-#include <cstring>
-#include <fcntl.h>
 #include <memory>
-#include <mutex>
-#include <poll.h>
 #include <stdexcept>
-#include <sys/epoll.h>
-#include <sys/eventfd.h>
-#include <sys/socket.h>
-#include <sys/uio.h>
-#include <sys/un.h>
-#include <thread>
-#include <unistd.h>
 #include <unordered_map>
 
-#include "h2.h"
-#include "pbwire.h"
+#include "loop_pool.h"
 
 namespace py = pybind11;
 using namespace kxdp;
 
 namespace {
 
-constexpr int STRATEGY_CDI_CRI = 0;
-constexpr int STRATEGY_CDI_ANNOTATIONS = 1;
-constexpr int STRATEGY_DEVICE_NODES = 2;
-constexpr size_t kMaxTimingSamples = 1u << 20;
-
-struct DeviceEntry {
-    std::vector<std::string> bdfs;
-    bool healthy = true;
-    std::string cdi_device;
-    std::string ann_key, ann_value;
-    std::string dev_path;
-};
-
-using Table = std::unordered_map<std::string, DeviceEntry>;
-
-struct AllocateConfig {
-    bool enabled = false;
-    std::string path;
-    int strategy = STRATEGY_CDI_CRI;
-    bool reject_unhealthy = true;
-    std::string cdi_kind, env_name, dev_root, devices_dir, required_driver;
-    std::vector<long> vendors;
-    bool timing = false;
-};
-
-enum class Kind { CONSTANT, WATCH, PYTHON, ALLOCATE };
-
-struct Method {
-    Kind kind;
-    std::string bytes;
-    py::object fn;
-};
-
-std::string link_base(int dirfd, const char* name) {
-    char buf[512];
-    ssize_t n = ::readlinkat(dirfd, name, buf, sizeof(buf) - 1);
-    if (n <= 0) return {};
-    buf[n] = 0;
-    const char* slash = std::strrchr(buf, '/');
-    return std::string(slash ? slash + 1 : buf);
-}
-
-long read_vendor(int dirfd) {
-    int fd = ::openat(dirfd, "vendor", O_RDONLY | O_CLOEXEC);
-    if (fd < 0) return -1;
-    char buf[64];
-    ssize_t n = ::read(fd, buf, sizeof(buf) - 1);
-    ::close(fd);
-    if (n <= 0) return -1;
-    buf[n] = 0;
-    errno = 0;
-    char* end = nullptr;
-    long v = std::strtol(buf, &end, 16);
-    if (errno || end == buf) return -1;
-    return v;
-}
-
-struct IoConn {
-    int fd;
-    h2::Conn h2;
-    size_t woff = 0;
-    size_t watching = 0;
-    bool want_write = false;
-    IoConn(int f, h2::App* app) : fd(f), h2(app) {}
-};
-
-class GrpcServer : public h2::App {
+class GrpcServer {
 public:
-    explicit GrpcServer(std::vector<std::string> paths)
-        : paths_(std::move(paths)) {}
-
-    ~GrpcServer() override {
-        if (thread_.joinable()) {
+    GrpcServer(std::vector<std::string> paths, int loops)
+        : pool_(std::move(paths), loops), ts_(loops, nullptr),
+          gstate_(loops) {
+        Hooks h;
+        h.thread_begin = [this](int i) {
+            if (_Py_IsFinalizing()) return;
+            gstate_[i] = PyGILState_Ensure();
+            ts_[i] = PyEval_SaveThread();
+        };
+        h.thread_end = [this](int i) {
+            if (ts_[i] && !_Py_IsFinalizing()) {
+                PyEval_RestoreThread(ts_[i]);
+                PyGILState_Release(gstate_[i]);
+            }
+            ts_[i] = nullptr;
+        };
+        h.unary = [this](int i, const std::string& path,
+                         const std::string& msg) {
+            return call_python(i, path, msg);
+        };
+        h.watch_change = [this](int i, long delta) {
+            GilHold gil(ts_[i]);
+            if (!gil.held || !on_watch_change_ || on_watch_change_.is_none())
+                return;
+            try {
+                on_watch_change_(delta);
+            } catch (py::error_already_set& e) {
+                e.restore();
+                PyErr_Clear();
+            }
+        };
+        h.reject = [this](int i, const std::string& err) {
+            GilHold gil(ts_[i]);
+            if (!gil.held || !on_reject_ || on_reject_.is_none()) return;
+            try {
+                on_reject_(err);
+            } catch (py::error_already_set& e) {
+                e.restore();
+                PyErr_Clear();
+            }
+        };
+        pool_.set_hooks(std::move(h));
+    }
+
+    ~GrpcServer() {
+        if (pool_.running()) {
             py::gil_scoped_release rel;
-            request_stop(0.0);
-            thread_.join();
-        }
-        methods_.clear();
+            pool_.stop(0.0);
+        }
+        unaries_.clear();
         on_reject_ = py::object();
         on_watch_change_ = py::object();
     }
 
     void register_constant(const std::string& path, const std::string& bytes) {
-        check_not_running();
-        methods_[path] = Method{Kind::CONSTANT, bytes, py::object()};
+        pool_.add_constant(path, bytes);
     }
     void register_watch(const std::string& path, py::object on_change) {
-        check_not_running();
-        methods_[path] = Method{Kind::WATCH, {}, py::object()};
+        pool_.add_watch(path);
         on_watch_change_ = std::move(on_change);
     }
     void register_unary(const std::string& path, py::object fn) {
-        check_not_running();
-        methods_[path] = Method{Kind::PYTHON, {}, std::move(fn)};
+        pool_.add_callback(path);
+        unaries_[path] = std::move(fn);
     }
     void configure_allocate(const std::string& path, const std::string& strategy,
                             bool reject_unhealthy, const std::string& cdi_kind,
@@ -130,22 +87,21 @@
                             const std::vector<long>& vendors,
                             const std::string& required_driver,
                             py::object on_reject, bool timing) {
-        check_not_running();
-        alloc_.enabled = true;
-        alloc_.path = path;
-        alloc_.strategy = strategy == "cdi-cri" ? STRATEGY_CDI_CRI
-                          : strategy == "cdi-annotations" ? STRATEGY_CDI_ANNOTATIONS
-                          : STRATEGY_DEVICE_NODES;
-        alloc_.reject_unhealthy = reject_unhealthy;
-        alloc_.cdi_kind = cdi_kind;
-        alloc_.env_name = env_name;
-        alloc_.dev_root = dev_root;
-        alloc_.devices_dir = devices_dir;
-        alloc_.vendors = vendors;
-        alloc_.required_driver = required_driver;
-        alloc_.timing = timing;
+        AllocateConfig a;
+        a.path = path;
+        a.strategy = strategy == "cdi-cri" ? STRATEGY_CDI_CRI
+                     : strategy == "cdi-annotations" ? STRATEGY_CDI_ANNOTATIONS
+                     : STRATEGY_DEVICE_NODES;
+        a.reject_unhealthy = reject_unhealthy;
+        a.cdi_kind = cdi_kind;
+        a.env_name = env_name;
+        a.dev_root = dev_root;
+        a.devices_dir = devices_dir;
+        a.vendors = vendors;
+        a.required_driver = required_driver;
+        a.timing = timing;
+        pool_.set_allocate(std::move(a));
         on_reject_ = std::move(on_reject);
-        methods_[path] = Method{Kind::ALLOCATE, {}, py::object()};
     }
 
     void update_table(const std::vector<std::tuple<
@@ -162,138 +118,36 @@
             e.dev_path = std::get<6>(d);
             (*t)[std::get<0>(d)] = std::move(e);
         }
-        std::lock_guard<std::mutex> g(table_mu_);
-        table_ = std::move(t);
-    }
-
-    void publish(const std::string& message) {
-        auto m = std::make_shared<const std::string>(message);
-        {
-            std::lock_guard<std::mutex> g(pub_mu_);
-            latest_ = std::move(m);
-            pub_gen_++;
-        }
-        wake();
-    }
-
-    void start() {
-        if (thread_.joinable()) throw std::runtime_error("server already started");
-        stop_.store(false);
-        ep_ = ::epoll_create1(EPOLL_CLOEXEC);
-        wake_fd_ = ::eventfd(0, EFD_NONBLOCK | EFD_CLOEXEC);
-        if (ep_ < 0 || wake_fd_ < 0) {
-            close_fds();
-            throw std::runtime_error("epoll/eventfd setup failed");
-        }
-        add_epoll(wake_fd_, EPOLLIN);
-        for (auto& path : paths_) {
-            sockaddr_un addr{};
-            addr.sun_family = AF_UNIX;
-            if (path.size() >= sizeof(addr.sun_path)) {
-                close_fds();
-                throw std::runtime_error("socket path too long: " + path);
-            }
-            std::memcpy(addr.sun_path, path.c_str(), path.size() + 1);
-            int fd = ::socket(AF_UNIX, SOCK_STREAM | SOCK_NONBLOCK | SOCK_CLOEXEC, 0);
-            if (fd < 0 || ::bind(fd, (sockaddr*)&addr, sizeof(addr)) < 0 ||
-                ::listen(fd, 128) < 0) {
-                std::string why = std::strerror(errno);
-                if (fd >= 0) ::close(fd);
-                close_fds();
-                throw std::runtime_error("cannot listen on " + path + ": " + why);
-            }
-            listeners_.push_back(fd);
-            bound_.push_back(path);
-            add_epoll(fd, EPOLLIN);
-        }
-        thread_ = std::thread([this] { run(); });
-    }
+        pool_.update_table(std::move(t));
+    }
+
+    void publish(const std::string& message) { pool_.publish(message); }
+
+    void start() { pool_.start(); }
 
     void stop(double grace) {
-        if (!thread_.joinable()) return;
+        if (!pool_.running()) return;
         py::gil_scoped_release rel;
-        request_stop(grace);
-        thread_.join();
-    }
-
-    bool running() const { return thread_.joinable(); }
+        pool_.stop(grace);
+    }
+
+    bool running() const { return pool_.running(); }
+    int loops() const { return pool_.loops(); }
 
     py::tuple stats() {
-        std::lock_guard<std::mutex> g(stat_mu_);
-        return py::make_tuple(allocations_, failures_, last_s_, total_s_);
+        PoolStats s = pool_.stats();
+        return py::make_tuple(s.allocations, s.failures, s.last_s, s.total_s);
     }
 
     std::vector<double> allocate_timing_us() {
-        std::lock_guard<std::mutex> g(stat_mu_);
-        return alloc_us_;
-    }
-
-    void on_rpc(h2::Conn& c, uint32_t sid, const std::string& path,
-                std::string& msg) override {
-        auto it = methods_.find(path);
-        if (it == methods_.end())
-            return c.reply_error(sid, h2::GRPC_UNIMPLEMENTED, "Method not found!");
-        Method& m = it->second;
-        switch (m.kind) {
-        case Kind::CONSTANT:
-            return c.reply_unary(sid, m.bytes);
-        case Kind::ALLOCATE:
-            return handle_allocate(c, sid, msg);
-        case Kind::WATCH: {
-            std::shared_ptr<const std::string> latest;
-            {
-                std::lock_guard<std::mutex> g(pub_mu_);
-                latest = latest_;
-            }
-            c.start_stream(sid);
-            if (latest) c.push_message(sid, *latest);
-            return;
-        }
-        case Kind::PYTHON:
-            return handle_python(c, sid, m, msg);
-        }
+        return pool_.allocate_timing_us();
+    }
+
+    std::vector<int> loop_connections() const {
+        return pool_.loop_connections();
     }
 
 private:
-    void check_not_running() {
-        if (thread_.joinable())
-            throw std::runtime_error("register methods before start()");
-    }
-
-    void wake() {
-        if (wake_fd_ >= 0) {
-            uint64_t one = 1;
-            ssize_t r = ::write(wake_fd_, &one, sizeof(one));
-            (void)r;
-        }
-    }
-
-    void request_stop(double grace) {
-        grace_s_ = grace;
-        stop_.store(true);
-        wake();
-    }
-
-    void add_epoll(int fd, uint32_t events) {
-        epoll_event ev{};
-        ev.events = events;
-        ev.data.fd = fd;
-        ::epoll_ctl(ep_, EPOLL_CTL_ADD, fd, &ev);
-    }
-
-    void close_fds() {
-        for (int fd : listeners_) ::close(fd);
-        listeners_.clear();
-        for (auto& p : bound_) ::unlink(p.c_str());
-        bound_.clear();
-        if (wake_fd_ >= 0) ::close(wake_fd_);
-        if (ep_ >= 0) ::close(ep_);
-        wake_fd_ = ep_ = -1;
-        if (dirfd_ >= 0) ::close(dirfd_);
-        dirfd_ = -1;
-        dirfd_table_ = nullptr;
-    }
-
     struct GilHold {
         PyThreadState*& ts;
         bool held = false;
@@ -308,395 +162,54 @@
         }
     };
 
-    void handle_python(h2::Conn& c, uint32_t sid, Method& m, std::string& msg) {
-        bool ok = false;
-        int status = h2::GRPC_UNKNOWN;
-        std::string payload;
-        {
-            GilHold gil(ts_);
-            if (!gil.held) {
-                status = h2::GRPC_UNAVAILABLE;
-                payload = "server shutting down";
+    UnaryResult call_python(int loop, const std::string& path,
+                            const std::string& msg) {
+        UnaryResult out;
+        GilHold gil(ts_[loop]);
+        if (!gil.held) {
+            out.status = h2::GRPC_UNAVAILABLE;
+            out.payload = "server shutting down";
+            return out;
+        }
+        try {
+            py::object r = unaries_.at(path)(py::bytes(msg));
+            if (py::isinstance<py::bytes>(r)) {
+                out.payload = r.cast<std::string>();
+                out.ok = true;
             } else {
-                try {
-                    py::object r = m.fn(py::bytes(msg));
-                    if (py::isinstance<py::bytes>(r)) {
-                        payload = r.cast<std::string>();
-                        ok = true;
-                    } else {
-                        auto t = r.cast<std::pair<int, std::string>>();
-                        status = t.first;
-                        payload = t.second;
-                    }
-                } catch (py::error_already_set& e) {
-                    try {
-                        payload = "Unexpected " +
-                                  py::str(e.type()).cast<std::string>() + ": " +
-                                  py::str(e.value()).cast<std::string>();
-                    } catch (...) {
-                        payload = "handler raised";
-                    }
-                    e.restore();
-                    PyErr_Clear();
-                } catch (std::exception& e) {
-                    payload = e.what();
-                }
-            }
-        }
-        if (ok) c.reply_unary(sid, payload);
-        else c.reply_error(sid, status, payload);
-    }
-
-    void report_watchers(IoConn& io, size_t now) {
-        if (now == io.watching) return;
-        long delta = (long)now - (long)io.watching;
-        io.watching = now;
-        GilHold gil(ts_);
-        if (!gil.held || !on_watch_change_ || on_watch_change_.is_none()) return;
-        try {
-            on_watch_change_(delta);
+                auto t = r.cast<std::pair<int, std::string>>();
+                out.status = t.first;
+                out.payload = t.second;
+            }
         } catch (py::error_already_set& e) {
+            try {
+                out.payload = "Unexpected " +
+                              py::str(e.type()).cast<std::string>() + ": " +
+                              py::str(e.value()).cast<std::string>();
+            } catch (...) {
+                out.payload = "handler raised";
+            }
             e.restore();
             PyErr_Clear();
-        }
-    }
-
-    void log_rejection(const std::string& err) {
-        GilHold gil(ts_);
-        if (!gil.held || !on_reject_ || on_reject_.is_none()) return;
-        try {
-            on_reject_(err);
-        } catch (py::error_already_set& e) {
-            e.restore();
-            PyErr_Clear();
-        }
-    }
-
-    bool open_devices_dir() {
-        if (dirfd_ >= 0) ::close(dirfd_);
-        dirfd_ = ::open(alloc_.devices_dir.c_str(),
-                        O_RDONLY | O_DIRECTORY | O_CLOEXEC);
-        return dirfd_ >= 0;
-    }
-
-    std::string revalidate(const std::string& gid, const DeviceEntry& dev) {
-        for (const auto& bdf : dev.bdfs) {
-            const int flags = O_RDONLY | O_DIRECTORY | O_CLOEXEC;
-            int dfd = ::openat(dirfd_, bdf.c_str(), flags);
-            if (dfd < 0) {
-                if (!open_devices_dir())
-                    return "cannot open " + alloc_.devices_dir;
-                dfd = ::openat(dirfd_, bdf.c_str(), flags);
-            }
-            if (dfd < 0) return "device " + bdf + " vanished";
-            std::string err;
-            if (link_base(dfd, "iommu_group") != gid) {
-                err = "device " + bdf + " no longer in IOMMU group " + gid;
-            } else {
-                long vendor = read_vendor(dfd);
-                if (vendor < 0 ||
-                    std::find(alloc_.vendors.begin(), alloc_.vendors.end(),
-                              vendor) == alloc_.vendors.end())
-                    err = "device " + bdf + " vendor not allowed";
-                else if (link_base(dfd, "driver") != alloc_.required_driver)
-                    err = "device " + bdf + " not bound to " +
-                          alloc_.required_driver;
-            }
-            ::close(dfd);
-            if (!err.empty()) return err;
-        }
-        return {};
-    }
-
-    std::string allocate_container(const Table& table,
-                                   const std::vector<std::string>& ids,
-                                   std::string& out) {
-        std::vector<const DeviceEntry*> devs;
-        devs.reserve(ids.size());
-        for (const auto& gid : ids) {
-            auto it = table.find(gid);
-            if (it == table.end()) return "unknown device id " + gid;
-            if (alloc_.reject_unhealthy && !it->second.healthy)
-                return "device " + gid + " is Unhealthy";
-            devs.push_back(&it->second);
-        }
-        if (dirfd_ < 0 || dirfd_table_ != &table) {
-            if (!open_devices_dir()) return "cannot open " + alloc_.devices_dir;
-            dirfd_table_ = &table;
-        }
-        for (size_t i = 0; i < ids.size(); i++) {
-            std::string err = revalidate(ids[i], *devs[i]);
-            if (!err.empty()) return err;
-        }
-        const bool cdi = alloc_.strategy != STRATEGY_DEVICE_NODES;
-        std::string bdfs;
-        for (auto* d : devs)
-            for (const auto& b : d->bdfs) {
-                if (!bdfs.empty()) bdfs.push_back(',');
-                bdfs += b;
-            }
-        static const std::string kVendorClass = "KUBERNETES_CDI_VENDOR_CLASS";
-        if (cdi && alloc_.env_name == kVendorClass) {
-            pb::put_map_entry(out, 1, alloc_.env_name, bdfs);
-        } else if (cdi && kVendorClass < alloc_.env_name) {
-            pb::put_map_entry(out, 1, kVendorClass, alloc_.cdi_kind);
-            pb::put_map_entry(out, 1, alloc_.env_name, bdfs);
-        } else {
-            pb::put_map_entry(out, 1, alloc_.env_name, bdfs);
-            if (cdi) pb::put_map_entry(out, 1, kVendorClass, alloc_.cdi_kind);
-        }
-        if (!cdi) {
-            auto spec = [&](const std::string& path) {
-                std::string s;
-                pb::put_bytes(s, 1, path);
-                pb::put_bytes(s, 2, path);
-                pb::put_bytes(s, 3, "rw", 2);
-                pb::put_bytes(out, 3, s);
-            };
-            if (!ids.empty()) spec(alloc_.dev_root + "/vfio/vfio");
-            for (auto* d : devs) spec(d->dev_path);
-        }
-        if (alloc_.strategy == STRATEGY_CDI_ANNOTATIONS)
-            for (auto* d : devs)
-                pb::put_map_entry(out, 4, d->ann_key, d->ann_value);
-        if (alloc_.strategy == STRATEGY_CDI_CRI)
-            for (auto* d : devs) pb::put_bytes(out, 5, d->cdi_device);
-        return {};
-    }
-
-    void handle_allocate(h2::Conn& c, uint32_t sid, const std::string& msg) {
-        auto t0 = std::chrono::steady_clock::now();
-        std::shared_ptr<const Table> table;
-        {
-            std::lock_guard<std::mutex> g(table_mu_);
-            table = table_;
-        }
-        std::vector<std::vector<std::string>> reqs;
-        if (!pb::parse_allocate_request(msg, reqs))
-            return c.reply_error(sid, h2::GRPC_INTERNAL,
-                                 "Exception deserializing request!");
-        static const Table kEmpty;
-        const Table& tbl = table ? *table : kEmpty;
-        std::string resp, err;
-        for (const auto& ids : reqs) {
-            std::string cresp;
-            err = allocate_container(tbl, ids, cresp);
-            if (!err.empty()) break;
-            pb::put_bytes(resp, 1, cresp);
-        }
-        if (!err.empty()) {
-            {
-                std::lock_guard<std::mutex> g(stat_mu_);
-                failures_++;
-            }
-            c.reply_error(sid, h2::GRPC_INVALID_ARGUMENT, err);
-            log_rejection(err);
-            return;
-        }
-        double dt = std::chrono::duration<double>(
-                        std::chrono::steady_clock::now() - t0).count();
-        {
-            std::lock_guard<std::mutex> g(stat_mu_);
-            allocations_++;
-            last_s_ = dt;
-            total_s_ += dt;
-            if (alloc_.timing && alloc_us_.size() < kMaxTimingSamples)
-                alloc_us_.push_back(dt * 1e6);
-        }
-        c.reply_unary(sid, resp);
-    }
-
-    void set_want_write(IoConn& io, bool on) {
-        if (io.want_write == on) return;
-        io.want_write = on;
-        epoll_event ev{};
-        ev.events = EPOLLIN | (on ? EPOLLOUT : 0);
-        ev.data.fd = io.fd;
-        ::epoll_ctl(ep_, EPOLL_CTL_MOD, io.fd, &ev);
-    }
-
-    bool flush(IoConn& io) {
-        std::string& out = io.h2.out();
-        while (io.woff < out.size()) {
-            iovec iov{(void*)(out.data() + io.woff), out.size() - io.woff};
-            msghdr mh{};
-            mh.msg_iov = &iov;
-            mh.msg_iovlen = 1;
-            ssize_t n = ::sendmsg(io.fd, &mh, MSG_NOSIGNAL);
-            if (n < 0) {
-                if (errno == EINTR) continue;
-                if (errno == EAGAIN || errno == EWOULDBLOCK) {
-                    set_want_write(io, true);
-                    return true;
-                }
-                return false;
-            }
-            io.woff += (size_t)n;
-        }
-        out.clear();
-        io.woff = 0;
-        set_want_write(io, false);
-        return !io.h2.want_close();
-    }
-
-    void close_conn(int fd) {
-        auto it = conns_.find(fd);
-        if (it == conns_.end()) return;
-        report_watchers(*it->second, 0);
-        ::epoll_ctl(ep_, EPOLL_CTL_DEL, fd, nullptr);
-        ::close(fd);
-        conns_.erase(it);
-    }
-
-    void on_readable(IoConn& io) {
-        ssize_t n = ::read(io.fd, rbuf_, sizeof(rbuf_));
-        if (n == 0) return close_conn(io.fd);
-        if (n < 0) {
-            if (errno == EAGAIN || errno == EINTR) return;
-            return close_conn(io.fd);
-        }
-        io.h2.feed((const uint8_t*)rbuf_, (size_t)n);
-        report_watchers(io, io.h2.watch_streams());
-        if (!flush(io)) close_conn(io.fd);
-    }
-
-    void deliver_publications() {
-        std::shared_ptr<const std::string> latest;
-        uint64_t gen;
-        {
-            std::lock_guard<std::mutex> g(pub_mu_);
-            latest = latest_;
-            gen = pub_gen_;
-        }
-        if (gen == pub_seen_ || !latest) return;
-        pub_seen_ = gen;
-        std::vector<int> done;
-        for (auto& kv : conns_) {
-            kv.second->h2.broadcast(*latest);
-            if (!flush(*kv.second)) done.push_back(kv.first);
-        }
-        for (int fd : done) close_conn(fd);
-    }
-
-    void shutdown_connections() {
-        for (int fd : listeners_) ::close(fd);
-        listeners_.clear();
-        for (auto& p : bound_) ::unlink(p.c_str());
-        bound_.clear();
-        for (auto& kv : conns_) kv.second->h2.begin_shutdown();
-        auto deadline = std::chrono::steady_clock::now() +
-                        std::chrono::duration<double>(grace_s_);
-        for (auto& kv : conns_) {
-            IoConn& io = *kv.second;
-            while (flush(io) && io.woff < io.h2.out().size()) {
-                auto left = std::chrono::duration_cast<std::chrono::milliseconds>(
-                    deadline - std::chrono::steady_clock::now()).count();
-                if (left <= 0) break;
-                pollfd p{io.fd, POLLOUT, 0};
-                if (::poll(&p, 1, (int)left) <= 0) break;
-            }
-            ::shutdown(io.fd, SHUT_WR);
-            while (::read(io.fd, rbuf_, sizeof(rbuf_)) > 0) {}
-            report_watchers(io, 0);
-            ::close(io.fd);
-        }
-        conns_.clear();
-    }
-
-    void run() {
-        PyGILState_STATE gstate = PyGILState_Ensure();
-        ts_ = PyEval_SaveThread();
-        epoll_event evs[64];
-        while (!stop_.load()) {
-            int n = ::epoll_wait(ep_, evs, 64, -1);
-            if (n < 0) {
-                if (errno == EINTR) continue;
-                break;
-            }
-            for (int i = 0; i < n && !stop_.load(); i++) {
-                int fd = evs[i].data.fd;
-                if (fd == wake_fd_) {
-                    uint64_t v;
-                    while (::read(wake_fd_, &v, sizeof(v)) > 0) {}
-                    deliver_publications();
-                    continue;
-                }
-                if (std::find(listeners_.begin(), listeners_.end(), fd) !=
-                    listeners_.end()) {
-                    for (;;) {
-                        int cfd = ::accept4(fd, nullptr, nullptr,
-                                            SOCK_NONBLOCK | SOCK_CLOEXEC);
-                        if (cfd < 0) break;
-                        auto io = std::make_unique<IoConn>(cfd, this);
-                        IoConn& ref = *io;
-                        conns_[cfd] = std::move(io);
-                        add_epoll(cfd, EPOLLIN);
-                        if (!flush(ref)) close_conn(cfd);
-                    }
-                    continue;
-                }
-                auto it = conns_.find(fd);
-                if (it == conns_.end()) continue;
-                IoConn& io = *it->second;
-                if (evs[i].events & EPOLLOUT) {
-                    if (!flush(io)) {
-                        close_conn(fd);
-                        continue;
-                    }
-                }
-                if (evs[i].events & (EPOLLIN | EPOLLHUP | EPOLLERR))
-                    on_readable(io);
-            }
-        }
-        shutdown_connections();
-        if (!_Py_IsFinalizing()) {
-            PyEval_RestoreThread(ts_);
-            PyGILState_Release(gstate);
-        }
-        ts_ = nullptr;
-        int ep = ep_, wfd = wake_fd_;
-        ep_ = wake_fd_ = -1;
-        ::close(ep);
-        ::close(wfd);
-        if (dirfd_ >= 0) ::close(dirfd_);
-        dirfd_ = -1;
-        dirfd_table_ = nullptr;
-    }
-
-    std::vector<std::string> paths_, bound_;
-    std::unordered_map<std::string, Method> methods_;
-    AllocateConfig alloc_;
+        } catch (std::exception& e) {
+            out.payload = e.what();
+        }
+        return out;
+    }
+
+    LoopPool pool_;
+    std::unordered_map<std::string, py::object> unaries_;
     py::object on_reject_, on_watch_change_;
-
-    std::mutex table_mu_;
-    std::shared_ptr<const Table> table_;
-    std::mutex pub_mu_;
-    std::shared_ptr<const std::string> latest_;
-    uint64_t pub_gen_ = 0;
-    uint64_t pub_seen_ = 0;
-
-    std::mutex stat_mu_;
-    uint64_t allocations_ = 0, failures_ = 0;
-    double last_s_ = 0.0, total_s_ = 0.0;
-    std::vector<double> alloc_us_;
-
-    std::thread thread_;
-    std::atomic<bool> stop_{false};
-    double grace_s_ = 1.0;
-    int ep_ = -1, wake_fd_ = -1;
-    std::vector<int> listeners_;
-    std::unordered_map<int, std::unique_ptr<IoConn>> conns_;
-    PyThreadState* ts_ = nullptr;
-    int dirfd_ = -1;
-    const Table* dirfd_table_ = nullptr;
-    char rbuf_[65536];
+    std::vector<PyThreadState*> ts_;
+    std::vector<PyGILState_STATE> gstate_;
 };
 
 }
 
 void kxdp_init_grpc_server(py::module_& m) {
     py::class_<GrpcServer>(m, "GrpcServer")
-        .def(py::init<std::vector<std::string>>(), py::arg("socket_paths"))
+        .def(py::init<std::vector<std::string>, int>(),
+             py::arg("socket_paths"), py::arg("loops") = 1)
         .def("register_constant", &GrpcServer::register_constant,
              py::arg("path"), py::arg("response"))
         .def("register_watch", &GrpcServer::register_watch, py::arg("path"),
@@ -716,5 +229,8 @@
         .def("stop", &GrpcServer::stop, py::arg("grace") = 1.0)
         .def("stats", &GrpcServer::stats)
         .def("allocate_timing_us", &GrpcServer::allocate_timing_us)
+        .def("loop_connections", &GrpcServer::loop_connections,
+             "open connections per loop thread")
+        .def_property_readonly("loops", &GrpcServer::loops)
         .def_property_readonly("running", &GrpcServer::running);
 }
diff --git a/setup.py b/setup.py
--- a/setup.py
+++ b/setup.py
@@ -66,7 +66,7 @@
                     sources=["native/xpu_native.cpp",
                              "native/xpu_grpc_server.cpp"],
                     depends=["native/h2.h", "native/hpack.h",
-                             "native/pbwire.h"],
+                             "native/pbwire.h", "native/loop_pool.h"],
                     include_dirs=[pybind11.get_include(), "native"],
                     extra_compile_args=["-O2", "-std=c++17"],
                     extra_link_args=["-pthread"],
```
